# ChainSafe/lumenos

Measured on AMD Instinct MI355X. Metric: prove_eval_seconds_16384x4096, lower is better.
Workload: dtype u64; 1 GPU; Encode+Commit+InnerProduct(r,b)+QueryCols 16384x4096 LogN=14 L=12 K=2 rhoInv=2 queries=309; parallelism=1 GPU: the whole job resident in HBM

## Files before the change

### lumenos_amd/csrc/lm_common.h

```cpp
#pragma once
#include <hip/hip_runtime.h>

#include <algorithm>
#include <cstdarg>
#include <cstdint>
#include <cstdio>
#include <map>
#include <memory>
#include <mutex>
#include <set>
#include <string>
#include <utility>
#include <vector>

#include "../../include/lumenos_hip.h"
#include "lm_arith.h"
#include "lm_dev.h"

#define LM_MAX_LIMBS LUMEN_MAX_LIMBS

struct lm_modmap {
    uint32_t period;
    uint8_t idx[LM_MAX_LIMBS];
};

struct lm_mods {
    mod_t m[LM_MAX_LIMBS];
};

struct lm_prof_entry {
    double total_ms = 0;
    uint64_t launches = 0;
    uint64_t units = 0;
};

struct lm_galois_key {
    lm_dev<u64> d_key;
    lm_dev<uint32_t> d_index;
    lm_dev<uint32_t> d_inv_index;
};

struct lumen_set {
    uint32_t count = 0;
    uint32_t nl = 0;
    uint32_t logw = 0;
    u64 *d = nullptr;
    size_t words = 0;
    bool owner = true;
    lumen_ctx *home = nullptr;
};

struct lm_shared {
    std::recursive_mutex mu;
    lm_dev<tw_t> tw_fwd;
    lm_dev<tw_t> tw_inv;
    std::vector<uint64_t> roots;
    uint32_t fieldN = 0;
    lm_dev<tw_t> scal;
    std::map<uint64_t, lm_galois_key> gkeys;
    std::map<std::string, std::shared_ptr<void>> ext;
};

struct lm_tuning {
    uint32_t ks_batch = 64;
    uint32_t ks_lanes = 0;
    int32_t ks_fused_digits = -1;
    uint32_t ks_close_fused = 1;
    uint32_t ks_c0_fold = 1;
    uint32_t debug = 0;
    uint32_t modup_tgroup = 3, moddown_tgroup = 1;
    uint32_t ks_placement = 6;
    uint32_t batch_chunks = 0;
    uint32_t dot_pairs = 0;
    uint32_t dot_parts = 0;
    uint32_t rccl_shared_device = 0;
};

struct lumen_ctx {
    lm_tuning tune;
    std::recursive_mutex mu;
    std::shared_ptr<lm_shared> sh;
    int device = 0;
    hipStream_t stream = nullptr;
    hipStream_t stream2 = nullptr;
    hipEvent_t ev_fork = nullptr, ev_join = nullptr;
    hipStream_t stream_aux = nullptr;
    hipEvent_t ev_aux = nullptr;
    hipEvent_t ev_xdep = nullptr;
    uint32_t aux_digests = 0;
    const u64 *aux_lo = nullptr, *aux_hi = nullptr;
    uint8_t *aux_host = nullptr;
    size_t aux_host_cap = 0;
    void *stage_host = nullptr;
    size_t stage_cap = 0;
    hipEvent_t ev_stage = nullptr;
    void *io_host[2] = {nullptr, nullptr};
    hipEvent_t ev_io[2] = {nullptr, nullptr};
    uint32_t logN = 0, N = 0, L = 0, K = 0;
    uint64_t T = 0;
    uint64_t mod[LM_MAX_LIMBS] = {0};
    uint64_t psi[LM_MAX_LIMBS] = {0};
    lm_mods mods;
    tw_t ninv[LM_MAX_LIMBS];
    std::vector<uint64_t> &roots;
    uint32_t &fieldN;
    std::map<uint64_t, lm_galois_key> &gkeys;
    std::map<std::string, std::shared_ptr<void>> &ext;
    uint64_t mul_counter = 0;
    std::map<std::string, lm_dev<unsigned char>> scratch;
    struct pool_block {
        void *p;
        hipEvent_t ready;
    };
    std::multimap<size_t, pool_block> pool;
    size_t pool_bytes = 0;
    std::set<const void *> lds_attr_done;
    bool prof = false;
    std::map<std::string, lm_prof_entry> prof_tab;
    struct pending_ev {
        std::string name;
        hipEvent_t a, b;
        uint64_t units;
    };
    std::vector<pending_ev> prof_pending;
    std::vector<hipEvent_t> ev_pool;
    hipEvent_t tm0 = nullptr, tm1 = nullptr;
    std::string err;
    explicit lumen_ctx(std::shared_ptr<lm_shared> s)
        : sh(std::move(s)), roots(sh->roots), fieldN(sh->fieldN), gkeys(sh->gkeys), ext(sh->ext) {}
};

static inline size_t lm_ctw(const lumen_ctx *ctx, const lumen_set *s);
#define LM_FULL_WIDTH(ctx, set, what) \
    LM_CHECK(ctx, (set)->logw == 0, "%s: lane-sharded set (1/%u of every limb) where a full-width set is required", what, 1u << (set)->logw)

#define LM_ENTER(ctx)                                             \
    std::lock_guard<std::recursive_mutex> lm_lock_((ctx)->mu);    \
    (void)hipSetDevice((ctx)->device);                            \
    (void)hipGetLastError()
#define LM_SHARED_LOCK(ctx) std::lock_guard<std::recursive_mutex> lm_shlock_((ctx)->sh->mu)

template <class T>
static inline std::shared_ptr<T> lm_ext_get(lumen_ctx *ctx, const std::string &key) {
    LM_SHARED_LOCK(ctx);
    auto it = ctx->ext.find(key);
    return it == ctx->ext.end() ? std::shared_ptr<T>() : std::static_pointer_cast<T>(it->second);
}
static inline void lm_ext_put(lumen_ctx *ctx, const std::string &key, std::shared_ptr<void> v) {
    LM_SHARED_LOCK(ctx);
    ctx->ext[key] = std::move(v);
}

static inline size_t lm_ctw(const lumen_ctx *ctx, const lumen_set *s) { return (size_t)2 * s->nl * (ctx->N >> s->logw); }

void lm_sync_all(lumen_ctx *ctx);
void *lm_stage(lumen_ctx *ctx, size_t bytes);
int lm_h2d_staged(lumen_ctx *ctx, void *dev, const void *host, size_t bytes);
bool lm_host_is_pinned(const void *p);
int lm_h2d(lumen_ctx *ctx, void *dev, const void *host, size_t bytes);
int lm_d2h(lumen_ctx *ctx, void *host, const void *dev, size_t bytes, bool wait);
int lm_h2d_rows(lumen_ctx *ctx, void *dev, size_t dpitch, const void *host, size_t spitch, size_t width, size_t height);

int lm_fail(lumen_ctx *ctx, const char *fmt, ...);
extern thread_local std::string lm_global_err;

#define LM_HIP(ctx, call)                                                                  \
    do {                                                                                   \
        hipError_t e_ = (call);                                                            \
        if (e_ != hipSuccess)                                                              \
            return lm_fail(ctx, "%s failed: %s (%s:%d)", #call, hipGetErrorString(e_),     \
                           __FILE__, __LINE__);                                            \
    } while (0)

#define LM_CHECK(ctx, cond, ...)                    \
    do {                                            \
        if (!(cond)) return lm_fail(ctx, __VA_ARGS__); \
    } while (0)

template <class... P, class... A>
static inline int lm_launch_flat(lumen_ctx *ctx, void (*kernel)(P...), size_t threads, A &&...args) {
    hipLaunchKernelGGL(kernel, dim3((uint32_t)((threads + 255) / 256)), dim3(256), 0, ctx->stream, std::forward<A>(args)...);
    LM_HIP(ctx, hipGetLastError());
    return 0;
}

struct lm_set_guard {
    lumen_ctx *ctx;
    lumen_set *s;
    lm_set_guard(lumen_ctx *c, lumen_set *x) : ctx(c), s(x) {}
    ~lm_set_guard() {
        if (s) lumen_set_destroy(ctx, s);
    }
    lumen_set *release() {
        lumen_set *r = s;
        s = nullptr;
        return r;
    }
    lm_set_guard(lm_set_guard &&o) : ctx(o.ctx), s(o.release()) {}
    lm_set_guard &operator=(const lm_set_guard &) = delete;
};

void lm_set_release_async(lumen_ctx *ctx, lumen_set *set);

void *lm_scratch(lumen_ctx *ctx, const char *name, size_t bytes);
void lm_scratch_adopt(lumen_ctx *ctx, const char *name, void *p, size_t bytes);

struct lm_prof_scope {
    lumen_ctx *ctx;
    const char *name;
    uint64_t units;
    hipEvent_t a = nullptr;
    lm_prof_scope(lumen_ctx *c, const char *n, uint64_t u);
    ~lm_prof_scope();
};
void lm_prof_resolve(lumen_ctx *ctx);

static inline uint64_t h_mulmod(uint64_t a, uint64_t b, uint64_t q) {
    return (uint64_t)(((u128)a * b) % q);
}
static inline uint64_t h_powmod(uint64_t a, uint64_t e, uint64_t q) {
    uint64_t r = 1 % q;
    a %= q;
    while (e) {
        if (e & 1) r = h_mulmod(r, a, q);
        a = h_mulmod(a, a, q);
        e >>= 1;
    }
    return r;
}
static inline uint64_t h_invmod(uint64_t a, uint64_t q) { return h_powmod(a, q - 2, q); }
static inline tw_t h_tw(uint64_t w, uint64_t q) {
    tw_t t;
    t.w = w;
    t.wp = (u64)((((u128)w) << 64) / q);
    return t;
}
static inline uint64_t h_r64_mod(uint64_t q) { return (uint64_t)((((u128)1) << 64) % q); }
static inline uint64_t h_p_mod(const lumen_ctx *ctx, uint64_t q) {
    uint64_t P = 1 % q;
    for (uint32_t a = 0; a < ctx->K; a++) P = h_mulmod(P, ctx->mod[ctx->L + a] % q, q);
    return P;
}
static inline uint32_t h_bitrev(uint32_t x, int bits) {
    uint32_t r = 0;
    for (int i = 0; i < bits; i++) r = (r << 1) | ((x >> i) & 1);
    return r;
}

int lm_launch_ntt(lumen_ctx *ctx, u64 *d, uint32_t npoly, const lm_modmap &map, bool inverse);
struct lm_ninv_t;
int lm_launch_ntt_strided(lumen_ctx *ctx, const u64 *src, size_t src_poly_stride, u64 *dst,
                          size_t dst_poly_stride, uint32_t npoly, const lm_modmap &map, bool inverse,
                          const char *prof_name, const lm_ninv_t *inv_scale = nullptr);
int lm_launch_ntt_subring(lumen_ctx *ctx, uint32_t logn, const tw_t *tw, tw_t ninv_scale, const u64 *src,
                          size_t src_poly_stride, u64 *dst, size_t dst_poly_stride, uint32_t npoly,
                          uint32_t mod_idx, bool inverse, const mod_t *explicit_mod = nullptr);
mod_t lm_make_mod(uint64_t q);
void lm_build_tw(uint64_t q, uint64_t psi, uint32_t logN, std::vector<tw_t> &fwd, std::vector<tw_t> &inv);
int lm_rescale_polys(lumen_ctx *ctx, const u64 *src, uint32_t nl, u64 *dst, uint32_t target,
                     uint32_t npoly, u64 *work, u64 *tbuf);
int lm_rescale_coef_ready(lumen_ctx *ctx);
int lm_rescale_polys_from_coef(lumen_ctx *ctx, const u64 *coef, uint32_t nl, u64 *dst, uint32_t target, uint32_t npoly);
lm_modmap lm_map_q(uint32_t nl);
lm_modmap lm_map_p(const lumen_ctx *ctx);
int lm_encode_dev(lumen_ctx *ctx, const lumen_set *matrix, const u64 *dzero, uint32_t rho_inv, lumen_set **encoded);
int lm_poly_eval_check(lumen_ctx *ctx, const uint64_t *values, uint32_t rows, uint32_t count, uint64_t first_column,
                       uint32_t cols, const char *what);
int lm_poly_eval_enqueue(lumen_ctx *ctx, const uint64_t *values, uint32_t rows, uint32_t count, uint64_t first_column,
                         uint32_t cols, uint64_t z, const char *what);
int lm_poly_eval_finish(lumen_ctx *ctx, uint64_t *partial);
hipEvent_t lm_ev_get(lumen_ctx *ctx);
```

### lumenos_amd/csrc/lm_ctx.hip

```cpp
#include <cstring>
#include <thread>

#include "lm_ntt_plan.h"

thread_local std::string lm_global_err;

int lm_fail(lumen_ctx *ctx, const char *fmt, ...) {
    char buf[1024];
    va_list ap;
    va_start(ap, fmt);
    vsnprintf(buf, sizeof(buf), fmt, ap);
    va_end(ap);
    if (ctx) ctx->err = buf;
    lm_global_err = buf;
    fprintf(stderr, "[lumenos_hip] error: %s\n", buf);
    return 1;
}

void *lm_scratch(lumen_ctx *ctx, const char *name, size_t bytes) {
    auto &e = ctx->scratch[name];
    if (e && e.count() >= bytes) return e.get();
    if (e) lm_sync_all(ctx);
    return e.alloc(ctx, bytes, name) ? nullptr : e.get();
}

void lm_scratch_adopt(lumen_ctx *ctx, const char *name, void *p, size_t bytes) {
    auto &e = ctx->scratch[name];
    if (e.get() == p) (void)e.release();
    if (e) lm_sync_all(ctx);
    e = lm_dev<unsigned char>((unsigned char *)p, bytes);
}

void lm_sync_all(lumen_ctx *ctx) {
    if (ctx->stream) hipStreamSynchronize(ctx->stream);
    if (ctx->stream2) hipStreamSynchronize(ctx->stream2);
    if (ctx->stream_aux) hipStreamSynchronize(ctx->stream_aux);
}

void *lm_stage(lumen_ctx *ctx, size_t bytes) {
    if (ctx->ev_stage) hipEventSynchronize(ctx->ev_stage);
    if (ctx->stage_cap < bytes) {
        if (ctx->stage_host) hipHostFree(ctx->stage_host);
        ctx->stage_host = nullptr, ctx->stage_cap = 0;
        if (hipHostMalloc(&ctx->stage_host, bytes, hipHostMallocDefault) != hipSuccess) {
            lm_fail(ctx, "hipHostMalloc(%zu) for host staging failed", bytes);
            return nullptr;
        }
        ctx->stage_cap = bytes;
    }
    return ctx->stage_host;
}

int lm_h2d_staged(lumen_ctx *ctx, void *dev, const void *host, size_t bytes) {
    void *h = lm_stage(ctx, bytes);
    if (!h) return 1;
    memcpy(h, host, bytes);
    LM_HIP(ctx, hipMemcpyAsync(dev, h, bytes, hipMemcpyHostToDevice, ctx->stream));
    LM_HIP(ctx, hipEventRecord(ctx->ev_stage, ctx->stream));
    return 0;
}

hipEvent_t lm_ev_get(lumen_ctx *ctx) {
    if (!ctx->ev_pool.empty()) {
        hipEvent_t e = ctx->ev_pool.back();
        ctx->ev_pool.pop_back();
        return e;
    }
    hipEvent_t e = nullptr;
    hipEventCreate(&e);
    return e;
}

lm_prof_scope::lm_prof_scope(lumen_ctx *c, const char *n, uint64_t u) : ctx(c), name(n), units(u) {
    if (!ctx->prof) return;
    a = lm_ev_get(ctx);
    hipEventRecord(a, ctx->stream);
}
lm_prof_scope::~lm_prof_scope() {
    if (!ctx->prof || !a) return;
    hipEvent_t b = lm_ev_get(ctx);
    hipEventRecord(b, ctx->stream);
    ctx->prof_pending.push_back({name, a, b, units});
}

void lm_prof_resolve(lumen_ctx *ctx) {
    if (ctx->prof_pending.empty()) return;
    for (auto &p : ctx->prof_pending) {
        float ms = 0;
        if (hipEventSynchronize(p.b) == hipSuccess && hipEventElapsedTime(&ms, p.a, p.b) == hipSuccess) {
            auto &e = ctx->prof_tab[p.name];
            e.total_ms += ms;
            e.launches += 1;
            e.units += p.units;
        } else {
            (void)hipGetLastError();
        }
        ctx->ev_pool.push_back(p.a);
        ctx->ev_pool.push_back(p.b);
    }
    ctx->prof_pending.clear();
}

lm_modmap lm_map_q(uint32_t nl) {
    lm_modmap m;
    m.period = nl;
    for (uint32_t i = 0; i < LM_MAX_LIMBS; i++) m.idx[i] = (uint8_t)(i < nl ? i : 0);
    return m;
}

lm_modmap lm_map_p(const lumen_ctx *ctx) {
    lm_modmap m;
    m.period = ctx->K;
    for (uint32_t i = 0; i < LM_MAX_LIMBS; i++) m.idx[i] = (uint8_t)(ctx->L + (i < ctx->K ? i : 0));
    return m;
}

mod_t lm_make_mod(uint64_t q) {
    mod_t m;
    m.q = q;
    m.qinv64 = (u64)((((u128)1) << 64) / q);
    u64 inv = 1;
    for (int it = 0; it < 6; it++) inv *= 2 - (u64)q * inv;
    m.qneg = (u64)0 - inv;
    u64 r = h_r64_mod(q);
    m.r2 = h_mulmod(r, r, q);
    return m;
}

void lm_build_tw(uint64_t q, uint64_t psi, uint32_t logN, std::vector<tw_t> &fwd, std::vector<tw_t> &inv) {
    uint32_t N = 1u << logN;
    fwd.resize(N);
    inv.resize(N);
    uint64_t psi_inv = h_invmod(psi, q), cf = 1, cb = 1;
    for (uint32_t j = 0; j < N; j++) {
        uint32_t r = h_bitrev(j, (int)logN);
        fwd[r] = h_tw(cf, q);
        inv[r] = h_tw(cb, q);
        cf = h_mulmod(cf, psi, q);
        cb = h_mulmod(cb, psi_inv, q);
    }
}

static void pool_drain(lumen_ctx *ctx) {
    for (auto &kv : ctx->pool) {
        hipFree(kv.second.p);
        if (kv.second.ready) ctx->ev_pool.push_back(kv.second.ready);
    }
    ctx->pool.clear();
    ctx->pool_bytes = 0;
}

static int ctx_private_init(lumen_ctx *ctx) {
    LM_HIP(ctx, hipSetDevice(ctx->device));
    LM_HIP(ctx, hipStreamCreate(&ctx->stream));
    LM_HIP(ctx, hipStreamCreate(&ctx->stream2));
    LM_HIP(ctx, hipEventCreateWithFlags(&ctx->ev_fork, hipEventDisableTiming));
    LM_HIP(ctx, hipEventCreateWithFlags(&ctx->ev_join, hipEventDisableTiming));
    LM_HIP(ctx, hipStreamCreate(&ctx->stream_aux));
    LM_HIP(ctx, hipEventCreateWithFlags(&ctx->ev_aux, hipEventDisableTiming));
    LM_HIP(ctx, hipEventCreateWithFlags(&ctx->ev_stage, hipEventDisableTiming));
    LM_HIP(ctx, hipEventCreateWithFlags(&ctx->ev_xdep, hipEventDisableTiming));
    LM_HIP(ctx, hipEventCreate(&ctx->tm0));
    LM_HIP(ctx, hipEventCreate(&ctx->tm1));
    return 0;
}

static int tuning_set(lm_tuning &t, const char *name, long v) {
    const std::string n(name ? name : "");
    auto in = [&](long lo, long hi) { return v >= lo && v <= hi; };
    if (n == "LUMEN_KS_BATCH") {
        if (!in(1, 4096)) return 2;
        t.ks_batch = (uint32_t)v;
    } else if (n == "LUMEN_KS_LANES") {
        if (!in(0, 2)) return 2;
        t.ks_lanes = (uint32_t)v;
    } else if (n == "LUMEN_KS_FUSED_DIGITS") {
        if (v > LM_MAX_LIMBS) return 2;
        t.ks_fused_digits = v >= 0 ? (int32_t)v : -1;
    } else if (n == "LUMEN_KS_CLOSE_FUSED") {
        if (!in(0, 1)) return 2;
        t.ks_close_fused = (uint32_t)v;
    } else if (n == "LUMEN_KS_C0_FOLD") {
        if (!in(0, 1)) return 2;
        t.ks_c0_fold = (uint32_t)v;
    } else if (n == "LUMEN_DEBUG") {
        t.debug = v != 0;
    } else if (n == "LUMEN_MODUP_TGROUP") {
        if (!in(1, 31)) return 2;
        t.modup_tgroup = (uint32_t)v;
    } else if (n == "LUMEN_MODDOWN_TGROUP") {
        if (!in(1, 31)) return 2;
        t.moddown_tgroup = (uint32_t)v;
    } else if (n == "LUMEN_KS_PLACEMENT") {
        if (!in(0, 32)) return 2;
        t.ks_placement = (uint32_t)v;
    } else if (n == "LUMEN_BATCH_CHUNKS") {
        if (!in(0, 4096)) return 2;
        t.batch_chunks = (uint32_t)v;
    } else if (n == "LUMEN_DOT_PAIRS") {
        if (v != 0 && v != 256 && v != 512) return 2;
        t.dot_pairs = (uint32_t)v;
    } else if (n == "LUMEN_DOT_PARTS") {
        if (!in(0, 256)) return 2;
        t.dot_parts = (uint32_t)v;
    } else {
        return 1;
    }
    return 0;
}
static void tuning_from_env(lm_tuning &t) {
    for (const char *n : {"LUMEN_KS_BATCH", "LUMEN_KS_LANES", "LUMEN_KS_FUSED_DIGITS", "LUMEN_KS_CLOSE_FUSED", "LUMEN_KS_C0_FOLD", "LUMEN_DEBUG",
                          "LUMEN_MODUP_TGROUP", "LUMEN_MODDOWN_TGROUP", "LUMEN_KS_PLACEMENT", "LUMEN_BATCH_CHUNKS", "LUMEN_DOT_PAIRS", "LUMEN_DOT_PARTS"}) {
        const char *e = getenv(n);
        if (e && *e && tuning_set(t, n, atol(e)))
            fprintf(stderr, "[lumenos_hip] %s=%s is out of range: ignored\n", n, e);
    }
}

extern "C" int lumen_ctx_set_tuning(lumen_ctx *ctx, const char *name, long value) {
    LM_CHECK(nullptr, ctx && name, "lumen_ctx_set_tuning: NULL argument");
    LM_ENTER(ctx);
    const int rc = tuning_set(ctx->tune, name, value);
    LM_CHECK(ctx, rc != 1, "unknown tuning switch %s", name);
    LM_CHECK(ctx, rc == 0, "tuning switch %s: value %ld is out of range (nothing changed)", name, value);
    return 0;
}

extern "C" int lumen_test_allow_shared_device_rccl(lumen_ctx *ctx, int on) {
    LM_CHECK(nullptr, ctx, "lumen_test_allow_shared_device_rccl: NULL ctx");
    LM_ENTER(ctx);
    ctx->tune.rccl_shared_device = on != 0;
    return 0;
}

extern "C" int lumen_ctx_wait(lumen_ctx *ctx, lumen_ctx *other) {
    LM_CHECK(nullptr, ctx && other, "lumen_ctx_wait: NULL argument");
    if (ctx == other) return 0;
    hipEvent_t ev;
    {
        LM_ENTER(other);
        LM_HIP(other, hipEventRecord(other->ev_xdep, other->stream));
        ev = other->ev_xdep;
    }
    LM_ENTER(ctx);
    LM_CHECK(ctx, ctx->device == other->device, "lumen_ctx_wait: contexts on devices %d and %d", ctx->device, other->device);
    LM_HIP(ctx, hipStreamWaitEvent(ctx->stream, ev, 0));
    return 0;
}

extern "C" int lumen_ctx_create(const lumen_params_desc *desc, lumen_ctx **out) {
    if (!desc || !out) return lm_fail(nullptr, "lumen_ctx_create: NULL argument");
    *out = nullptr;
    LM_CHECK(nullptr, desc->abi_version == LUMEN_ABI_VERSION, "ABI version mismatch: got %u want %u",
             desc->abi_version, LUMEN_ABI_VERSION);
    LM_CHECK(nullptr, lm_logn_supported(desc->log_n) || lm_logn_split_supported(desc->log_n),
             "log_n %u unsupported: kernels are instantiated for N = 2^8 and 2^10..2^14, and the server's path and the key "
             "switch for N = 2^15",
             desc->log_n);
    LM_CHECK(nullptr, desc->num_q >= 1 && desc->num_q + desc->num_p <= LM_MAX_LIMBS,
             "bad limb counts L=%u K=%u", desc->num_q, desc->num_p);
    int ndev = 0;
    if (hipGetDeviceCount(&ndev) != hipSuccess || ndev == 0)
        return lm_fail(nullptr, "no HIP device visible: the lumenos HIP path has no CPU fallback");
    LM_CHECK(nullptr, desc->device >= 0 && desc->device < ndev, "device %d out of range (have %d)",
             desc->device, ndev);
    std::unique_ptr<lumen_ctx, void (*)(lumen_ctx *)> guard(new lumen_ctx(std::make_shared<lm_shared>()),
                                                            lumen_ctx_destroy);
    lumen_ctx *ctx = guard.get();
    tuning_from_env(ctx->tune);
    ctx->device = desc->device;
    ctx->logN = desc->log_n;
    ctx->N = 1u << desc->log_n;
    ctx->L = desc->num_q;
    ctx->K = desc->num_p;
    ctx->T = desc->plaintext_modulus;
    uint32_t LK = ctx->L + ctx->K, N = ctx->N;
    uint64_t two_n = 2ull * N;
    for (uint32_t i = 0; i < LK; i++) {
        uint64_t q = desc->moduli[i], psi = desc->psi[i];
        const uint64_t qmax = UINT64_MAX / lm_q_bound_factor(desc->log_n);
        if (q < (1ull << 20) || q > qmax || (q & (two_n - 1)) != 1)
            return lm_fail(nullptr, "modulus %u (%llu) must be == 1 mod 2N and below %llu", i,
                           (unsigned long long)q, (unsigned long long)qmax);
        if (h_powmod(psi, N, q) != q - 1)
            return lm_fail(nullptr, "psi[%u] is not a primitive 2N-th root of unity", i);
        ctx->mod[i] = q;
        ctx->psi[i] = psi;
        ctx->mods.m[i] = lm_make_mod(q);
        ctx->ninv[i] = h_tw(h_invmod(N % q, q), q);
    }
    for (uint32_t i = LK; i < LM_MAX_LIMBS; i++) ctx->mods.m[i] = ctx->mods.m[0];
    if (int rc = ctx_private_init(ctx)) return rc;
    std::vector<tw_t> f, b, fwd, inv;
    for (uint32_t i = 0; i < LK; i++) {
        lm_build_tw(ctx->mod[i], ctx->psi[i], ctx->logN, f, b);
        fwd.insert(fwd.end(), f.begin(), f.end());
        inv.insert(inv.end(), b.begin(), b.end());
    }
    lm_layout_tw(fwd, ctx->logN);
    lm_layout_tw(inv, ctx->logN);
    if (ctx->sh->tw_fwd.upload(ctx, fwd, "the forward twiddles") || ctx->sh->tw_inv.upload(ctx, inv, "the inverse twiddles")) return 1;
    *out = guard.release();
    return 0;
}

extern "C" int lumen_ctx_clone(lumen_ctx *src, lumen_ctx **out) {
    if (!src || !out) return lm_fail(nullptr, "lumen_ctx_clone: NULL argument");
    *out = nullptr;
    LM_ENTER(src);
    std::unique_ptr<lumen_ctx, void (*)(lumen_ctx *)> guard(new lumen_ctx(src->sh), lumen_ctx_destroy);
    lumen_ctx *ctx = guard.get();
    ctx->tune = src->tune;
    ctx->device = src->device;
    ctx->logN = src->logN, ctx->N = src->N, ctx->L = src->L, ctx->K = src->K, ctx->T = src->T;
    memcpy(ctx->mod, src->mod, sizeof(ctx->mod));
    memcpy(ctx->psi, src->psi, sizeof(ctx->psi));
    ctx->mods = src->mods;
    memcpy(ctx->ninv, src->ninv, sizeof(ctx->ninv));
    if (int rc = ctx_private_init(ctx)) {
        src->err = ctx->err;
        return rc;
    }
    *out = guard.release();
    return 0;
}

extern "C" void lumen_ctx_destroy(lumen_ctx *ctx) {
    if (!ctx) return;
    {
        LM_ENTER(ctx);
        lm_sync_all(ctx);
        ctx->scratch.clear();
        pool_drain(ctx);
        lm_prof_resolve(ctx);
        for (hipEvent_t e : ctx->ev_pool) hipEventDestroy(e);
        if (ctx->tm0) hipEventDestroy(ctx->tm0);
        if (ctx->tm1) hipEventDestroy(ctx->tm1);
        if (ctx->aux_host) hipHostFree(ctx->aux_host);
        if (ctx->stage_host) hipHostFree(ctx->stage_host);
        for (int i = 0; i < 2; i++) {
            if (ctx->io_host[i]) hipHostFree(ctx->io_host[i]);
            if (ctx->ev_io[i]) hipEventDestroy(ctx->ev_io[i]);
        }
        if (ctx->ev_stage) hipEventDestroy(ctx->ev_stage);
        if (ctx->ev_xdep) hipEventDestroy(ctx->ev_xdep);
        if (ctx->ev_aux) hipEventDestroy(ctx->ev_aux);
        if (ctx->stream_aux) hipStreamDestroy(ctx->stream_aux);
        if (ctx->ev_fork) hipEventDestroy(ctx->ev_fork);
        if (ctx->ev_join) hipEventDestroy(ctx->ev_join);
        if (ctx->stream2) hipStreamDestroy(ctx->stream2);
        if (ctx->stream) hipStreamDestroy(ctx->stream);
        ctx->sh.reset();
    }
    delete ctx;
}

extern "C" int lumen_ctx_trim(lumen_ctx *ctx) {
    LM_CHECK(nullptr, ctx, "lumen_ctx_trim: NULL ctx");
    LM_ENTER(ctx);
    LM_CHECK(ctx, !ctx->aux_digests, "lumen_ctx_trim: a lumen_leaf_digests_begin job is in flight");
    lm_sync_all(ctx);
    for (auto it = ctx->scratch.begin(); it != ctx->scratch.end();) {
        if (it->first == "digests_async" || it->first == "group_digests") {
            ++it;
            continue;
        }
        it = ctx->scratch.erase(it);
    }
    pool_drain(ctx);
    return 0;
}

extern "C" int lumen_ctx_scratch_info(lumen_ctx *ctx, const char *name, void **ptr, size_t *bytes) {
    LM_CHECK(nullptr, ctx && name && ptr, "lumen_ctx_scratch_info: NULL argument");
    LM_ENTER(ctx);
    auto it = ctx->scratch.find(name);
    *ptr = it == ctx->scratch.end() ? nullptr : it->second.get();
    if (bytes) *bytes = it == ctx->scratch.end() ? 0 : it->second.count();
    return 0;
}

extern "C" const char *lumen_last_error(const lumen_ctx *ctx) {
    return ctx ? ctx->err.c_str() : lm_global_err.c_str();
}

extern "C" int lumen_sync(lumen_ctx *ctx) {
    LM_CHECK(nullptr, ctx, "lumen_sync: NULL ctx");
    LM_ENTER(ctx);
    LM_HIP(ctx, hipStreamSynchronize(ctx->stream));
    return 0;
}

extern "C" uint64_t lumen_mul_counter(const lumen_ctx *ctx) { return ctx ? ctx->mul_counter : 0; }

extern "C" int lumen_set_create(lumen_ctx *ctx, uint32_t count, uint32_t num_limbs, lumen_set **out) {
    return lumen_set_create_lanes(ctx, count, num_limbs, 0, out);
}

extern "C" int lumen_set_create_lanes(lumen_ctx *ctx, uint32_t count, uint32_t num_limbs, uint32_t log_world,
                                      lumen_set **out) {
    LM_CHECK(nullptr, ctx && out, "lumen_set_create: NULL argument");
    LM_ENTER(ctx);
    LM_CHECK(ctx, num_limbs >= 1 && num_limbs <= ctx->L, "num_limbs %u out of range [1,%u]", num_limbs, ctx->L);
    LM_CHECK(ctx, log_world <= 6 && (ctx->N >> log_world) >= 64, "a lane shard of 1/%u of N = %u is narrower than 64 coefficients",
             1u << log_world, ctx->N);
    lumen_set *s = new lumen_set();
    s->count = count;
    s->nl = num_limbs;
    s->logw = log_world;
    s->words = (size_t)count * 2 * num_limbs * (ctx->N >> log_world);
    s->home = ctx;
    if (s->words) {
        const size_t bytes = s->words * sizeof(u64);
        auto it = ctx->pool.find(bytes);
        if (it != ctx->pool.end()) {
            s->d = (u64 *)it->second.p;
            if (hipEvent_t ready = it->second.ready) {
                (void)hipStreamWaitEvent(ctx->stream, ready, 0);
                (void)hipStreamWaitEvent(ctx->stream2, ready, 0);
                (void)hipStreamWaitEvent(ctx->stream_aux, ready, 0);
                ctx->ev_pool.push_back(ready);
            }
            ctx->pool.erase(it);
            ctx->pool_bytes -= bytes;
        } else {
            hipError_t e = hipMalloc((void **)&s->d, bytes);
            if (e != hipSuccess && !ctx->pool.empty()) {
                (void)hipGetLastError();
                lm_sync_all(ctx);
                pool_drain(ctx);
                e = hipMalloc((void **)&s->d, bytes);
            }
            if (e != hipSuccess) {
                (void)hipGetLastError();
                delete s;
                return lm_fail(ctx, "hipMalloc(%zu bytes) for a %u x %u-limb set failed: %s", bytes, count,
                               num_limbs, hipGetErrorString(e));
            }
        }
    }
    *out = s;
    return 0;
}

extern "C" void lumen_set_destroy(lumen_ctx *ctx, lumen_set *set) {
    if (!set) return;
    if (ctx) {
        LM_ENTER(ctx);
        hipStreamSynchronize(ctx->stream);
        hipStreamSynchronize(ctx->stream2);
        if (ctx->aux_digests && set->d && set->d < ctx->aux_hi && set->d + set->words > ctx->aux_lo)
            hipStreamSynchronize(ctx->stream_aux);
        if (set->owner && set->d) {
            const size_t bytes = set->words * sizeof(u64);
            if (ctx == set->home && ctx->pool_bytes + bytes <= ((size_t)96 << 30)) {
                ctx->pool.emplace(bytes, lumen_ctx::pool_block{set->d, nullptr});
                ctx->pool_bytes += bytes;
            } else {
                hipFree(set->d);
            }
        }
    } else if (set->owner && set->d) {
        hipFree(set->d);
    }
    delete set;
}

void lm_set_release_async(lumen_ctx *ctx, lumen_set *set) {
    if (!set) return;
    LM_ENTER(ctx);
    const size_t bytes = set->words * sizeof(u64);
    const bool hashing = ctx->aux_digests && set->d && set->d < ctx->aux_hi && set->d + set->words > ctx->aux_lo;
    if (!set->owner || !set->d || ctx != set->home || hashing || ctx->pool_bytes + bytes > ((size_t)96 << 30)) {
        lumen_set_destroy(ctx, set);
        return;
    }
    hipEvent_t ready = lm_ev_get(ctx);
    bool ok = ready && hipEventRecord(ctx->ev_join, ctx->stream2) == hipSuccess &&
              hipStreamWaitEvent(ctx->stream, ctx->ev_join, 0) == hipSuccess && hipEventRecord(ready, ctx->stream) == hipSuccess;
    if (!ok) {
        (void)hipGetLastError();
        if (ready) ctx->ev_pool.push_back(ready);
        lumen_set_destroy(ctx, set);
        return;
    }
    ctx->pool.emplace(bytes, lumen_ctx::pool_block{set->d, ready});
    ctx->pool_bytes += bytes;
    delete set;
}

extern "C" int lumen_set_slice(lumen_ctx *ctx, const lumen_set *set, uint32_t first, uint32_t n,
                               lumen_set **view) {
    LM_CHECK(nullptr, ctx && set && view, "lumen_set_slice: NULL argument");
    LM_ENTER(ctx);
    LM_CHECK(ctx, (uint64_t)first + n <= set->count, "slice [%u,%u) exceeds set of %u", first, first + n, set->count);
    lumen_set *v = new lumen_set();
    const size_t ctw = lm_ctw(ctx, set);
    v->count = n;
    v->nl = set->nl;
    v->logw = set->logw;
    v->d = set->d + (size_t)first * ctw;
    v->words = (size_t)n * ctw;
    v->owner = false;
    *view = v;
    return 0;
}

extern "C" uint32_t lumen_set_count(const lumen_set *set) { return set ? set->count : 0; }
extern "C" uint32_t lumen_set_limbs(const lumen_set *set) { return set ? set->nl : 0; }
extern "C" uint32_t lumen_set_log_world(const lumen_set *set) { return set ? set->logw : 0; }
extern "C" void *lumen_set_device_ptr(const lumen_set *set) { return set ? set->d : nullptr; }

extern "C" void *lumen_host_alloc(size_t bytes) {
    void *p = nullptr;
    if (hipHostMalloc(&p, bytes ? bytes : 1, hipHostMallocDefault) != hipSuccess) {
        (void)hipGetLastError();
        lm_fail(nullptr, "hipHostMalloc(%zu) failed", bytes);
        return nullptr;
    }
    return p;
}
extern "C" void lumen_host_free(void *p) {
    if (p) hipHostFree(p);
}

static int host_limbs_move(uint64_t *flat, uint64_t *const *limbs, size_t n, size_t words, uint32_t threads, bool gather) {
    if (!n || !words) return 0;
    const size_t bytes = words * sizeof(uint64_t);
    size_t nthr = threads ? threads : std::max(1u, std::min(16u, std::thread::hardware_concurrency()));
    nthr = std::min(nthr, n);
    auto work = [=](size_t lo, size_t hi) {
        for (size_t i = lo; i < hi; i++) {
            if (gather) memcpy(flat + i * words, limbs[i], bytes);
            else memcpy(limbs[i], flat + i * words, bytes);
        }
    };
    if (nthr == 1) {
        work(0, n);
        return 0;
    }
    std::vector<std::thread> th;
    for (size_t t = 0; t < nthr; t++) th.emplace_back(work, n * t / nthr, n * (t + 1) / nthr);
    for (auto &x : th) x.join();
    return 0;
}
extern "C" int lumen_host_gather(uint64_t *dst, const uint64_t *const *limbs, size_t n, size_t words, uint32_t threads) {
    LM_CHECK(nullptr, (dst && limbs) || !n, "lumen_host_gather: NULL argument");
    for (size_t i = 0; i < n; i++) LM_CHECK(nullptr, limbs[i], "lumen_host_gather: limb %zu is NULL", i);
    return host_limbs_move(dst, const_cast<uint64_t *const *>(limbs), n, words, threads, true);
}
extern "C" int lumen_host_scatter(const uint64_t *src, uint64_t *const *limbs, size_t n, size_t words, uint32_t threads) {
    LM_CHECK(nullptr, (src && limbs) || !n, "lumen_host_scatter: NULL argument");
    for (size_t i = 0; i < n; i++) LM_CHECK(nullptr, limbs[i], "lumen_host_scatter: limb %zu is NULL", i);
    return host_limbs_move(const_cast<uint64_t *>(src), limbs, n, words, threads, false);
}

bool lm_host_is_pinned(const void *p) {
    hipPointerAttribute_t a;
    if (hipPointerGetAttributes(&a, p) != hipSuccess) {
        (void)hipGetLastError();
        return false;
    }
    return a.type == hipMemoryTypeHost;
}

#define LM_IO_CHUNK ((size_t)64 << 20)
static void par_memcpy(void *dst, const void *src, size_t bytes) {
    const size_t nthr = bytes >= ((size_t)8 << 20) ? 4 : 1;
    if (nthr == 1) {
        memcpy(dst, src, bytes);
        return;
    }
    std::thread th[4];
    const size_t part = (bytes / nthr + 63) & ~(size_t)63;
    for (size_t t = 0; t < nthr; t++) {
        const size_t lo = std::min(bytes, t * part), hi = std::min(bytes, lo + part);
        th[t] = std::thread([=] { memcpy((char *)dst + lo, (const char *)src + lo, hi - lo); });
    }
    for (size_t t = 0; t < nthr; t++) th[t].join();
}

static int io_buffers(lumen_ctx *ctx) {
    for (int i = 0; i < 2; i++) {
        if (!ctx->io_host[i]) LM_HIP(ctx, hipHostMalloc(&ctx->io_host[i], LM_IO_CHUNK, hipHostMallocDefault));
        if (!ctx->ev_io[i]) LM_HIP(ctx, hipEventCreateWithFlags(&ctx->ev_io[i], hipEventDisableTiming));
    }
    return 0;
}

int lm_h2d(lumen_ctx *ctx, void *dev, const void *host, size_t bytes) {
    char *dst = (char *)dev;
    if (bytes <= ((size_t)1 << 20) || lm_host_is_pinned(host)) {
        LM_HIP(ctx, hipMemcpyAsync(dst, host, bytes, hipMemcpyHostToDevice, ctx->stream));
    } else {
        if (int rc = io_buffers(ctx)) return rc;
        int i = 0;
        for (size_t off = 0; off < bytes; off += LM_IO_CHUNK, i ^= 1) {
            const size_t len = std::min(LM_IO_CHUNK, bytes - off);
            LM_HIP(ctx, hipEventSynchronize(ctx->ev_io[i]));
            par_memcpy(ctx->io_host[i], (const char *)host + off, len);
            LM_HIP(ctx, hipMemcpyAsync(dst + off, ctx->io_host[i], len, hipMemcpyHostToDevice, ctx->stream));
            LM_HIP(ctx, hipEventRecord(ctx->ev_io[i], ctx->stream));
        }
    }
    LM_HIP(ctx, hipStreamSynchronize(ctx->stream));
    return 0;
}

int lm_h2d_rows(lumen_ctx *ctx, void *dev, size_t dpitch, const void *host, size_t spitch, size_t width, size_t height) {
    char *dst = (char *)dev;
    const char *src = (const char *)host;
    if (!width || !height) return 0;
    if (width * height <= ((size_t)1 << 20) || lm_host_is_pinned(host)) {
        LM_HIP(ctx, hipMemcpy2DAsync(dst, dpitch, src, spitch, width, height, hipMemcpyHostToDevice, ctx->stream));
    } else {
        LM_CHECK(ctx, width <= LM_IO_CHUNK, "lm_h2d_rows: a row of %zu bytes exceeds the bounce buffer", width);
        if (int rc = io_buffers(ctx)) return rc;
        const size_t per = LM_IO_CHUNK / width;
        int i = 0;
        for (size_t r = 0; r < height; r += per, i ^= 1) {
            const size_t nr = std::min(per, height - r);
            LM_HIP(ctx, hipEventSynchronize(ctx->ev_io[i]));
            if (spitch == width)
                par_memcpy(ctx->io_host[i], src + r * spitch, nr * width);
            else
                for (size_t k = 0; k < nr; k++) memcpy((char *)ctx->io_host[i] + k * width, src + (r + k) * spitch, width);
            LM_HIP(ctx, hipMemcpy2DAsync(dst + r * dpitch, dpitch, ctx->io_host[i], width, width, nr, hipMemcpyHostToDevice,
                                         ctx->stream));
            LM_HIP(ctx, hipEventRecord(ctx->ev_io[i], ctx->stream));
        }
    }
    LM_HIP(ctx, hipStreamSynchronize(ctx->stream));
    return 0;
}

extern "C" int lumen_set_upload(lumen_ctx *ctx, lumen_set *set, uint32_t first, uint32_t n,
                                const uint64_t *host) {
    LM_CHECK(nullptr, ctx && set && host, "lumen_set_upload: NULL argument");
    LM_ENTER(ctx);
    LM_CHECK(ctx, (uint64_t)first + n <= set->count, "upload range [%u,%u) exceeds set of %u", first, first + n, set->count);
    const size_t ctw = lm_ctw(ctx, set), bytes = (size_t)n * ctw * sizeof(u64);
    return lm_h2d(ctx, set->d + (size_t)first * ctw, host, bytes);
}

int lm_d2h(lumen_ctx *ctx, void *host, const void *dev, size_t bytes, bool wait) {
    const char *src = (const char *)dev;
    if (bytes <= ((size_t)1 << 20) || lm_host_is_pinned(host)) {
        LM_HIP(ctx, hipMemcpyAsync(host, src, bytes, hipMemcpyDeviceToHost, ctx->stream));
        if (wait || !lm_host_is_pinned(host)) LM_HIP(ctx, hipStreamSynchronize(ctx->stream));
        return 0;
    }
    if (int rc = io_buffers(ctx)) return rc;
    const size_t nchunks = (bytes + LM_IO_CHUNK - 1) / LM_IO_CHUNK;
    auto issue = [&](size_t k) -> int {
        const size_t off = k * LM_IO_CHUNK, len = std::min(LM_IO_CHUNK, bytes - off);
        LM_HIP(ctx, hipMemcpyAsync(ctx->io_host[k & 1], src + off, len, hipMemcpyDeviceToHost, ctx->stream));
        LM_HIP(ctx, hipEventRecord(ctx->ev_io[k & 1], ctx->stream));
        return 0;
    };
    if (nchunks)
        if (int rc = issue(0)) return rc;
    for (size_t k = 0; k < nchunks; k++) {
        if (k + 1 < nchunks)
            if (int rc = issue(k + 1)) return rc;
        const size_t off = k * LM_IO_CHUNK, len = std::min(LM_IO_CHUNK, bytes - off);
        LM_HIP(ctx, hipEventSynchronize(ctx->ev_io[k & 1]));
        par_memcpy((char *)host + off, ctx->io_host[k & 1], len);
    }
    return 0;
}

extern "C" int lumen_set_download(lumen_ctx *ctx, const lumen_set *set, uint32_t first, uint32_t n,
                                  uint64_t *host) {
    LM_CHECK(nullptr, ctx && set && host, "lumen_set_download: NULL argument");
    LM_ENTER(ctx);
    LM_CHECK(ctx, (uint64_t)first + n <= set->count, "download range [%u,%u) exceeds set of %u", first, first + n, set->count);
    const size_t ctw = lm_ctw(ctx, set), bytes = (size_t)n * ctw * sizeof(u64);
    return lm_d2h(ctx, host, set->d + (size_t)first * ctw, bytes, true);
}

__global__ void k_fill_random(u64 *d, size_t words, uint32_t N, uint32_t nl, lm_mods mods, u64 seed) {
    size_t i = (size_t)blockIdx.x * blockDim.x + threadIdx.x;
    size_t stride = (size_t)gridDim.x * blockDim.x;
    for (; i < words; i += stride) {
        uint32_t limb = (uint32_t)((i / N) % nl);
        u64 z = seed + 0x9e3779b97f4a7c15ull * (u64)(i + 1);
        z = (z ^ (z >> 30)) * 0xbf58476d1ce4e5b9ull;
        z = (z ^ (z >> 27)) * 0x94d049bb133111ebull;
        z ^= z >> 31;
        d[i] = lm_reduce(z, mods.m[limb].q, mods.m[limb].qinv64);
    }
}

extern "C" int lumen_set_fill_random(lumen_ctx *ctx, lumen_set *set, uint64_t seed) {
    LM_CHECK(nullptr, ctx && set, "lumen_set_fill_random: NULL argument");
    LM_ENTER(ctx);
    if (!set->words) return 0;
    hipLaunchKernelGGL(k_fill_random, dim3(2048), dim3(256), 0, ctx->stream, set->d, set->words,
                       ctx->N >> set->logw, set->nl, ctx->mods, (u64)seed);
    LM_HIP(ctx, hipGetLastError());
    return 0;
}

extern "C" int lumen_timer_start(lumen_ctx *ctx) {
    LM_CHECK(nullptr, ctx, "NULL ctx");
    LM_ENTER(ctx);
    LM_HIP(ctx, hipEventRecord(ctx->tm0, ctx->stream));
    return 0;
}

extern "C" int lumen_timer_stop(lumen_ctx *ctx, float *elapsed_ms) {
    LM_CHECK(nullptr, ctx && elapsed_ms, "NULL argument");
    LM_ENTER(ctx);
    LM_HIP(ctx, hipEventRecord(ctx->tm1, ctx->stream));
    LM_HIP(ctx, hipEventSynchronize(ctx->tm1));
    LM_HIP(ctx, hipEventElapsedTime(elapsed_ms, ctx->tm0, ctx->tm1));
    return 0;
}

extern "C" int lumen_prof_enable(lumen_ctx *ctx, int on) {
    LM_CHECK(nullptr, ctx, "NULL ctx");
    LM_ENTER(ctx);
    if (!on) lm_prof_resolve(ctx);
    ctx->prof = on != 0;
    return 0;
}

extern "C" int lumen_prof_reset(lumen_ctx *ctx) {
    LM_CHECK(nullptr, ctx, "NULL ctx");
    LM_ENTER(ctx);
    lm_prof_resolve(ctx);
    ctx->prof_tab.clear();
    return 0;
}

extern "C" size_t lumen_prof_names(lumen_ctx *ctx, char *buf, size_t cap) {
    if (!ctx) return 0;
    LM_ENTER(ctx);
    lm_prof_resolve(ctx);
    std::string all;
    for (auto &kv : ctx->prof_tab) {
        if (!all.empty()) all += ",";
        all += kv.first;
    }
    if (buf && cap) {
        size_t n = std::min(cap - 1, all.size());
        memcpy(buf, all.data(), n);
        buf[n] = 0;
    }
    return all.size();
}

extern "C" int lumen_prof_read(lumen_ctx *ctx, const char *kernel, double *total_ms,
                               uint64_t *launches, uint64_t *units) {
    LM_CHECK(nullptr, ctx && kernel, "NULL argument");
    LM_ENTER(ctx);
    lm_prof_resolve(ctx);
    auto it = ctx->prof_tab.find(kernel);
    lm_prof_entry e;
    if (it != ctx->prof_tab.end()) e = it->second;
    if (total_ms) *total_ms = e.total_ms;
    if (launches) *launches = e.launches;
    if (units) *units = e.units;
    return 0;
}
```

### lumenos_amd/csrc/lm_innersum.hip

```cpp
#include <algorithm>

#include "lm_ks_host.h"

__global__ __launch_bounds__(256) void k_acc_canon(u64 *__restrict__ acc, size_t pairs, uint32_t logN, uint32_t L, lm_mods mods) {
    const size_t stride = (size_t)gridDim.x * blockDim.x;
    for (size_t g = (size_t)blockIdx.x * blockDim.x + threadIdx.x; g < pairs; g += stride) {
        const u64 q = mods.m[(uint32_t)((g >> (logN - 1)) % L)].q;
        ulonglong2 v = *reinterpret_cast<ulonglong2 *>(acc + 2 * g);
        v.x = lm_csub(v.x, q), v.y = lm_csub(v.y, q);
        *reinterpret_cast<ulonglong2 *>(acc + 2 * g) = v;
    }
}

__global__ __launch_bounds__(256) void k_lazy_gather(const u64 *__restrict__ u, const u64 *__restrict__ cur, u64 *__restrict__ lazy,
                                                     const uint32_t *__restrict__ index, uint32_t B, uint32_t L, uint32_t K,
                                                     uint32_t pshift, uint32_t logN, uint32_t first, lm_mods mods) {
    const uint32_t N = 1u << logN, nq = L * 2 * B;
    const size_t total = (size_t)2 * B * (L + K) * (N / 2), stride = (size_t)gridDim.x * blockDim.x;
    for (size_t g = (size_t)blockIdx.x * blockDim.x + threadIdx.x; g < total; g += stride) {
        const uint32_t j = (uint32_t)(g & (N / 2 - 1)) * 2, limb = (uint32_t)(g >> (logN - 1));
        const uint32_t t = limb < nq ? limb / (2 * B) : L + (limb - nq) % K;
        const uint32_t pw = limb < nq ? limb % (2 * B) : (limb - nq) / K;
        const bool with_c = t < L && (pw & 1) == (u ? 0u : 1u);
        if (!u && !with_c) continue;
        const u64 q = mods.m[ks_mod_at(t, L, pshift)].q;
        const size_t o = ((size_t)limb << logN) + j;
        uint2 p;
        p.x = j, p.y = j + 1;
        if (index) p = *reinterpret_cast<const uint2 *>(index + j);
        ulonglong2 v;
        v.x = v.y = 0;
        if (!first) v = *reinterpret_cast<const ulonglong2 *>(lazy + o);
        if (u) v.x += u[((size_t)limb << logN) + p.x], v.y += u[((size_t)limb << logN) + p.y];
        if (with_c) {
            const u64 *c = cur + (((size_t)pw * L + t) << logN);
            v.x += c[p.x], v.y += c[p.y];
        }
        v.x = lm_csub(lm_csub(v.x, 2 * q), q), v.y = lm_csub(lm_csub(v.y, 2 * q), q);
        *reinterpret_cast<ulonglong2 *>(lazy + o) = v;
    }
}

namespace {

int acc_canon(lumen_ctx *ctx, u64 *acc, size_t words, uint32_t L) {
    if (!words) return 0;
    hipLaunchKernelGGL(k_acc_canon, dim3(2048), dim3(256), 0, ctx->stream, acc, words / 2, ctx->logN, L, ctx->mods);
    LM_HIP(ctx, hipGetLastError());
    return 0;
}


bool is_plain(const lumen_ctx *ctx, uint32_t batch, uint32_t n) { return batch == 1 && n && !(n & (n - 1)) && n <= ctx->N; }

template <class Fn>
int sum_walk(const lumen_ctx *ctx, uint32_t batch, uint32_t n, Fn &&fn) {
    if (is_plain(ctx, batch, n)) {
        uint64_t gal[64];
        const uint32_t cnt = lumen_inner_sum_galois_elements(ctx, n, gal);
        for (uint32_t r = 0; r < cnt; r++)
            if (int rc = fn((uint64_t)0, gal[r])) return rc;
        return 0;
    }
    for (uint32_t i = 0, j = n; j > 1; i++, j >>= 1) {
        const uint64_t term = (j & 1) ? lumen_galois_element(ctx, (int64_t)((uint64_t)(n - (n & ((2u << i) - 1))) * batch)) : 0;
        if (int rc = fn(term, lumen_galois_element(ctx, (int64_t)((uint64_t)batch << i)))) return rc;
    }
    return 0;
}

struct SumPlan {
    struct Step {
        const lm_galois_key *dbl = nullptr, *term = nullptr;
        uint64_t dbl_el = 0;
    } it[32];
    uint32_t cnt = 0;
    uint64_t last_el = 0;
    bool lazy = false;
};

int sum_plan(lumen_ctx *ctx, uint32_t batch, uint32_t n, SumPlan *p) {
    return sum_walk(ctx, batch, n, [&](uint64_t term, uint64_t dbl) {
        SumPlan::Step &st = p->it[p->cnt++];
        if (term) {
            if (int rc = ks_find_key(ctx, term, &st.term)) return rc;
            p->lazy = true;
        }
        p->last_el = st.dbl_el = dbl;
        return ks_find_key(ctx, dbl, &st.dbl);
    });
}

int general_check(lumen_ctx *ctx, uint32_t batch, uint32_t n, const char *what) {
    LM_CHECK(ctx, batch >= 1 && n >= 1, "%s: batch size %u and length %u must both be at least 1", what, batch, n);
    LM_CHECK(ctx, ctx->K >= 1, "parameters have no special primes: key switching unavailable");
    LM_CHECK(ctx, ctx->K <= 2, "key switching supports 1 or 2 special primes (have %u)", ctx->K);
    if (is_plain(ctx, batch, n)) return 0;
    LM_CHECK(ctx, (uint64_t)batch * n <= ctx->N / 2, "%s: batch size %u x length %u spans beyond the slot row of %u slots", what, batch, n,
             ctx->N / 2);
    return 0;
}

}


int lazy_blocks(lumen_ctx *ctx, const KsRun &run, u64 **lazy) {
    const size_t bytes = (size_t)run.Bmax * 2 * (ctx->L + ctx->K) * ctx->N * 8;
    lazy[0] = (u64 *)lm_scratch(ctx, "ks_lazy", bytes);
    lazy[1] = run.lanes > 1 ? (u64 *)lm_scratch(ctx, "ks_lazy_b", bytes) : lazy[0];
    return lazy[0] && lazy[1] ? 0 : 1;
}

static int lazy_gather(lumen_ctx *ctx, const u64 *u, const u64 *cur, u64 *lazy, const uint32_t *index, bool first, uint32_t B, KsTables *tb) {
    lm_prof_scope ps(ctx, "ks_lazy_gather", (uint64_t)B);
    hipLaunchKernelGGL(k_lazy_gather, dim3(2048), dim3(256), 0, ctx->stream, u, cur, lazy, index, B, tb->nl, ctx->K, ctx->L - tb->nl,
                       ctx->logN, first ? 1u : 0u, ctx->mods);
    LM_HIP(ctx, hipGetLastError());
    return 0;
}

int identity_tables(lumen_ctx *ctx, std::shared_ptr<lm_galois_key> *out) {
    static const char *const NAME = "ks_identity";
    LM_SHARED_LOCK(ctx);
    auto gk = lm_ext_get<lm_galois_key>(ctx, NAME);
    if (!gk) {
        gk = std::make_shared<lm_galois_key>();
        std::vector<uint32_t> index(ctx->N);
        for (uint32_t i = 0; i < ctx->N; i++) index[i] = i;
        if (gk->d_index.upload(ctx, index, "the identity's index table") || gk->d_inv_index.upload(ctx, index, "the identity's index table"))
            return 1;
        lm_ext_put(ctx, NAME, gk);
    }
    *out = std::move(gk);
    return 0;
}

int lazy_close(lumen_ctx *ctx, const u64 *cur, u64 *out, u64 *lazy, uint32_t B, KsTables *tb, const KsScratch &s) {
    std::shared_ptr<lm_galois_key> id;
    if (int rc = identity_tables(ctx, &id)) return rc;
    if (int rc = lazy_gather(ctx, nullptr, cur, lazy, nullptr, false, B, tb)) return rc;
    if (int rc = rotate_p_to_coef(ctx, lazy, B, tb)) return rc;
    KsScratch sl = s;
    sl.u = lazy;
    return rotate_store(ctx, cur, out, B, *id, tb, sl);
}

namespace {

int inner_sum_batch(lumen_ctx *ctx, u64 *acc, uint32_t B, const SumPlan &plan, KsTables *tb, const KsScratch &s, u64 *lazy,
                    u64 *close_out, u64 *fold_s = nullptr) {
    LM_CHECK(ctx, !close_out || (plan.cnt && !plan.lazy), "InnerSum has no rotation to close");
    LM_CHECK(ctx, !fold_s || (close_out && ks_fold_serves(ctx, tb, plan.cnt)),
             "the c0 fold cannot hold the lifts of %u rotations of %u bits in 192", plan.cnt, tb->lift_bits);
    u64 *cur = acc, *other = s.acc2;
    bool first = true;
    for (uint32_t r = 0; r < plan.cnt; r++) {
        const SumPlan::Step &st = plan.it[r];
        if (int rc = rotate_decompose(ctx, cur, B, tb, s)) return rc;
        if (fold_s) {
            const u64 *s_in = r ? fold_s + ((r - 1) & 1) * ks_fold_words(ctx, B) : nullptr;
            u64 *s_out = fold_s + (r & 1) * ks_fold_words(ctx, B);
            if (r + 1 == plan.cnt) return rotate_close_fold(ctx, cur, close_out, B, *st.dbl, st.dbl_el, tb, s, s_in, s_out);
            if (int rc = rotate_add_fold(ctx, cur, other, B, *st.dbl, st.dbl_el, tb, s, s_in, s_out)) return rc;
            std::swap(cur, other);
            continue;
        }
        if (st.term) {
            if (int rc = rotate_mac(ctx, cur, B, *st.term, tb, s)) return rc;
            if (int rc = lazy_gather(ctx, s.u, cur, lazy, st.term->d_index.get(), first, B, tb)) return rc;
            first = false;
        }
        if (close_out && r + 1 == plan.cnt)
            return rotate_close(ctx, cur, close_out, B, *st.dbl, plan.last_el, tb, s);
        if (int rc = rotate_add(ctx, cur, other, B, *st.dbl, tb, s)) return rc;
        std::swap(cur, other);
    }
    if (plan.lazy) {
        if (int rc = lazy_close(ctx, cur, other, lazy, B, tb, s)) return rc;
        std::swap(cur, other);
    }
    if (cur != acc)
        LM_HIP(ctx, hipMemcpyAsync(acc, cur, (size_t)B * 2 * tb->nl * ctx->N * 8, hipMemcpyDeviceToDevice, ctx->stream));
    return 0;
}

int check_inner_sum_level(lumen_ctx *ctx, const lumen_set *in, const char *what) {
    LM_FULL_WIDTH(ctx, in, what);
    LM_CHECK(ctx, in->nl == ctx->L, "%s is implemented at the top level only (set has %u of %u limbs)", what,
             in->nl, ctx->L);
    return 0;
}

int inner_sum_run(lumen_ctx *ctx, const lumen_set *in, uint32_t batch, uint32_t n, const char *general, lumen_set **out) {
    if (general) {
        if (int rc = general_check(ctx, batch, n, general)) return rc;
    } else {
        LM_CHECK(ctx, is_plain(ctx, batch, n), "InnerSum length %u is not a power of two <= N", n);
    }
    KsRun run;
    if (int rc = ks_run_open(ctx, in->count, in->nl, is_plain(ctx, batch, n) ? 1 : 2, false, &run)) return rc;
    SumPlan plan;
    if (in->count)
        if (int rc = sum_plan(ctx, batch, n, &plan)) return rc;
    lumen_set *o = nullptr;
    if (int rc = lumen_set_create(ctx, in->count, in->nl, &o)) return rc;
    lm_set_guard og(ctx, o);
    if (in->words)
        LM_HIP(ctx, hipMemcpyAsync(o->d, in->d, in->words * 8, hipMemcpyDeviceToDevice, ctx->stream));
    if (int rc = ks_run_scratch(ctx, &run)) return rc;
    u64 *lazy[2] = {nullptr, nullptr};
    if (plan.lazy)
        if (int rc = lazy_blocks(ctx, run, lazy)) return rc;
    const size_t ctw = (size_t)2 * in->nl * ctx->N;
    auto batch_fn = [&](uint32_t, uint32_t first, uint32_t B, const KsScratch &s, u64 *) {
        return inner_sum_batch(ctx, o->d + (size_t)first * ctw, B, plan, run.tb, s, lazy[&s == &run.s[1]], nullptr);
    };
    if (int rc = ks_run(ctx, run, in->count, ctw, batch_fn)) return rc;
    if (!plan.lazy)
        if (int rc = acc_canon(ctx, o->d, o->words, in->nl)) return rc;
    *out = og.release();
    return 0;
}

int matrix_inner_sum_run(lumen_ctx *ctx, const lumen_set *matrix, const uint64_t *pt, uint32_t rows, const char *general,
                         lumen_set **out) {
    if (general) {
        if (int rc = general_check(ctx, 1, rows, general)) return rc;
    } else {
        LM_CHECK(ctx, is_plain(ctx, 1, rows), "rows=%u is not a power of two <= N", rows);
    }
    KsRun run;
    if (int rc = ks_run_open(ctx, matrix->count, matrix->nl, 2, true, &run)) return rc;
    SumPlan plan;
    if (matrix->count)
        if (int rc = sum_plan(ctx, 1, rows, &plan)) return rc;
    u64 *ptT = nullptr;
    if (int rc = upload_ptT(ctx, pt, matrix->nl, &ptT)) return rc;
    const uint32_t N = ctx->N, L = matrix->nl, target = std::min<uint32_t>(2, L);
    lumen_set *o = nullptr;
    if (int rc = lumen_set_create(ctx, matrix->count, target, &o)) return rc;
    lm_set_guard og(ctx, o);
    const size_t ctw = (size_t)2 * L * N, octw = (size_t)2 * target * N;
    if (int rc = ks_run_scratch(ctx, &run)) return rc;
    u64 *lazy[2] = {nullptr, nullptr};
    if (plan.lazy)
        if (int rc = lazy_blocks(ctx, run, lazy)) return rc;
    u64 *work = (u64 *)lm_scratch(ctx, "rescale_work", run.group_bytes);
    u64 *tbuf = (u64 *)lm_scratch(ctx, "rescale_t", (size_t)run.group * 2 * N * 8);
    if (!work || !tbuf) return 1;
    bool close = false;
    if (L > target && rows > 1 && ctx->tune.ks_close_fused && !plan.lazy && !lm_is_split(ctx->logN)) {
        const int rc = lm_rescale_coef_ready(ctx);
        if (rc && rc != 2) return rc;
        close = rc == 0;
    }
    u64 *fold_s[2] = {nullptr, nullptr};
    if (close && ctx->tune.ks_c0_fold && ks_fold_serves(ctx, run.tb, plan.cnt)) {
        const size_t bytes = 2 * ks_fold_words(ctx, run.Bmax) * 8;
        fold_s[0] = (u64 *)lm_scratch(ctx, "ks_fold_s", bytes);
        fold_s[1] = run.lanes > 1 ? (u64 *)lm_scratch(ctx, "ks_fold_s_b", bytes) : fold_s[0];
        if (!fold_s[0] || !fold_s[1]) return 1;
    }
    auto batch_fn = [&](uint32_t g0, uint32_t first, uint32_t B, const KsScratch &s, u64 *a) {
        if (int rc = launch_mul_plain(ctx, matrix->d + (size_t)(g0 + first) * ctw, a, ptT, (size_t)B * ctw, L, B))
            return rc;
        const int lane = &s == &run.s[1];
        return inner_sum_batch(ctx, a, B, plan, run.tb, s, lazy[lane], close ? work + (size_t)first * ctw : nullptr, fold_s[lane]);
    };
    auto end_of_group = [&](uint32_t g0, uint32_t gn) {
        if (close)
            return lm_rescale_polys_from_coef(ctx, work, L, o->d + (size_t)g0 * octw, target, gn * 2);
        if (L > target) return lm_rescale_polys(ctx, run.acc, L, o->d + (size_t)g0 * octw, target, gn * 2, work, tbuf);
        if (!plan.lazy)
            if (int rc = acc_canon(ctx, run.acc, (size_t)gn * ctw, L)) return rc;
        LM_HIP(ctx, hipMemcpyAsync(o->d + (size_t)g0 * octw, run.acc, (size_t)gn * ctw * 8, hipMemcpyDeviceToDevice, ctx->stream));
        return 0;
    };
    if (int rc = ks_run(ctx, run, matrix->count, ctw, batch_fn, end_of_group)) return rc;
    *out = og.release();
    return 0;
}

}

extern "C" int lumen_inner_sum_general(lumen_ctx *ctx, const lumen_set *in, uint32_t batch_size, uint32_t n, lumen_set **out) {
    LM_CHECK(nullptr, ctx && in && out, "lumen_inner_sum_general: NULL argument");
    LM_ENTER(ctx);
    if (int rc = check_level_of_chain(ctx, in, "InnerSum")) return rc;
    return inner_sum_run(ctx, in, batch_size, n, "lumen_inner_sum_general", out);
}

extern "C" int lumen_matrix_inner_sum_general(lumen_ctx *ctx, const lumen_set *matrix, const uint64_t *pt, uint32_t rows,
                                              lumen_set **out) {
    LM_CHECK(nullptr, ctx && matrix && pt && out, "lumen_matrix_inner_sum_general: NULL argument");
    LM_ENTER(ctx);
    if (int rc = check_level_of_chain(ctx, matrix, "matrixInnerSumEval")) return rc;
    return matrix_inner_sum_run(ctx, matrix, pt, rows, "lumen_matrix_inner_sum_general", out);
}

extern "C" uint32_t lumen_inner_sum_general_elements(const lumen_ctx *ctx, uint32_t batch_size, uint32_t n, uint64_t *gal_els) {
    if (!ctx || !gal_els) return 0;
    if (!is_plain(ctx, batch_size, n) && (!batch_size || !n || (uint64_t)batch_size * n > ctx->N / 2)) return 0;
    uint32_t cnt = 0;
    sum_walk(ctx, batch_size, n, [&](uint64_t term, uint64_t dbl) {
        for (uint64_t g : {term, dbl})
            if (g > 1 && std::find(gal_els, gal_els + cnt, g) == gal_els + cnt) gal_els[cnt++] = g;
        return 0;
    });
    return cnt;
}

extern "C" int lumen_inner_sum(lumen_ctx *ctx, const lumen_set *in, uint32_t n, lumen_set **out) {
    LM_CHECK(nullptr, ctx && in && out, "lumen_inner_sum: NULL argument");
    LM_ENTER(ctx);
    if (int rc = check_inner_sum_level(ctx, in, "InnerSum")) return rc;
    return inner_sum_run(ctx, in, 1, n, nullptr, out);
}

extern "C" int lumen_inner_sum_at_level(lumen_ctx *ctx, const lumen_set *in, uint32_t n, lumen_set **out) {
    LM_CHECK(nullptr, ctx && in && out, "lumen_inner_sum_at_level: NULL argument");
    LM_ENTER(ctx);
    if (int rc = check_level_of_chain(ctx, in, "InnerSum")) return rc;
    return inner_sum_run(ctx, in, 1, n, nullptr, out);
}

extern "C" int lumen_matrix_inner_sum(lumen_ctx *ctx, const lumen_set *matrix, const uint64_t *pt,
                                      uint32_t rows, lumen_set **out) {
    LM_CHECK(nullptr, ctx && matrix && pt && out, "lumen_matrix_inner_sum: NULL argument");
    LM_ENTER(ctx);
    if (int rc = check_inner_sum_level(ctx, matrix, "matrixInnerSumEval")) return rc;
    return matrix_inner_sum_run(ctx, matrix, pt, rows, nullptr, out);
}

extern "C" int lumen_matrix_inner_sum_at_level(lumen_ctx *ctx, const lumen_set *matrix, const uint64_t *pt,
                                               uint32_t rows, lumen_set **out) {
    LM_CHECK(nullptr, ctx && matrix && pt && out, "lumen_matrix_inner_sum_at_level: NULL argument");
    LM_ENTER(ctx);
    if (int rc = check_level_of_chain(ctx, matrix, "matrixInnerSumEval")) return rc;
    return matrix_inner_sum_run(ctx, matrix, pt, rows, nullptr, out);
}
```

### lumenos_amd/csrc/lm_keyswitch.hip

```cpp
#include <cstdlib>
#include <cstring>

#include "lm_ks_host.h"

__device__ __forceinline__ u32 bx_v(u128 A, u128 M, u64 y0, u64 y1, u64 m0, u64 m1) {
    const u128 D1 = A >= M ? A - M : M - A, D2 = 2 * M - A;
    if ((u64)(D1 >> 64) >= 8 && (u64)(D2 >> 64) >= 8) return A >= M ? 1u : 0u;
    double vf = 0.0;
    vf += (double)y0 / (double)m0;
    vf += (double)y1 / (double)m1;
    return (u32)(u64)vf;
}

__device__ __forceinline__ void pack_pair(u64 a, u64 b, u64 m0, u64 m1, u128 M, u64 &hi, u64 &lo) {
    u64 l1, h1, l2, h2;
    mul128(a, m1, l1, h1);
    mul128(b, m0, l2, h2);
    const u128 A = (((u128)h1 << 64) | l1) + (((u128)h2 << 64) | l2);
    const u32 v = bx_v(A, M, a, b, m0, m1);
    const u128 W = A + (v == 0 ? 2 * M : (v == 1 ? M : (u128)0));
    hi = (u64)(W >> LM_W_SPLIT), lo = (u64)W & ((1ull << LM_W_SPLIT) - 1);
}

__global__ __launch_bounds__(256) void k_pack_v(u64 *__restrict__ y, size_t poly_stride, uint32_t npoly,
                                                uint32_t ngroups, uint32_t group_limbs, uint32_t first_mod,
                                                uint32_t nlimbs_total, uint32_t logN, lm_mods mods) {
    const uint32_t N = 1u << logN;
    const size_t total = (size_t)npoly * ngroups * (N / 2), stride = (size_t)gridDim.x * blockDim.x;
    for (size_t g = (size_t)blockIdx.x * blockDim.x + threadIdx.x; g < total; g += stride) {
        const uint32_t i = (uint32_t)(g & (N / 2 - 1)) * 2;
        const uint32_t grp = (uint32_t)((g >> (logN - 1)) % ngroups), p = (uint32_t)((g >> (logN - 1)) / ngroups);
        const uint32_t l0 = grp * group_limbs;
        if (l0 + 1 >= nlimbs_total) continue;
        u64 *y0 = y + (size_t)p * poly_stride + (size_t)l0 * N + i;
        const ulonglong2 av = *reinterpret_cast<const ulonglong2 *>(y0);
        const ulonglong2 bv = *reinterpret_cast<const ulonglong2 *>(y0 + N);
        const u64 m0 = mods.m[first_mod + l0].q, m1 = mods.m[first_mod + l0 + 1].q;
        u64 Ml, Mh;
        mul128(m0, m1, Ml, Mh);
        const u128 M = ((u128)Mh << 64) | Ml;
        ulonglong2 hv, lv;
#pragma unroll
        for (int e = 0; e < 2; e++) {
            const u64 a = e ? av.y : av.x, b = e ? bv.y : bv.x;
            u64 hi, lo;
            pack_pair(a, b, m0, m1, M, hi, lo);
            if (e) hv.y = hi, lv.y = lo;
            else hv.x = hi, lv.x = lo;
        }
        *reinterpret_cast<ulonglong2 *>(y0) = hv;
        *reinterpret_cast<ulonglong2 *>(y0 + N) = lv;
    }
}

template <int LOGN>
__global__ LM_GEOM_BOUNDS(lm_geom_lds(LOGN)) void k_intt_pack(const u64 *__restrict__ acc, u64 *coef, uint32_t B,
                                                                  uint32_t L, uint32_t nf, lm_mods mods,
                                                                  lm_ninv_t yscale, const tw_t *__restrict__ tw_all) {
    extern __shared__ __attribute__((aligned(16))) u64 sm[];
    constexpr uint32_t N = 1u << LOGN;
    const uint32_t tid = threadIdx.x;
    if (blockIdx.x >= B * nf) {
        const uint32_t k = blockIdx.x - B * nf, l = 2 * nf + k / B, b = k % B;
        const u64 *p = acc + (((size_t)b * 2 + 1) * L + l) * N;
        u64 *o = coef + ((size_t)b * L + l) * N;
        const lm_qc q = lm_make_qc(mods.m[l]);
        const tw_t sc = yscale.t[l];
        auto ld = [&](uint32_t i0, u64 *v, int count) { lm_load_run(p, i0, v, count); };
        auto st = [&](uint32_t i, u64 v) { o[i] = lm_shoup_cs(v, sc, q.q, q.nq); };
        lm_ntt_inverse<LOGN>(sm, tw_all + (size_t)l * N, q, tid, ld, st);
        return;
    }
    const uint32_t d = blockIdx.x / B, b = blockIdx.x % B;
    const uint32_t l0 = 2 * d, l1 = l0 + 1;
    const u64 *c1 = acc + ((size_t)b * 2 + 1) * L * N;
    u64 *o0 = coef + ((size_t)b * L + l0) * N;
    const lm_qc q0 = lm_make_qc(mods.m[l0]);
    const tw_t s0 = yscale.t[l0];
    {
        const u64 *p = c1 + (size_t)l0 * N;
        auto ld = [&](uint32_t i0, u64 *v, int count) { lm_load_run(p, i0, v, count); };
        auto st = [&](uint32_t i, u64 v) { o0[i] = lm_shoup_cs(v, s0, q0.q, q0.nq); };
        lm_ntt_inverse<LOGN>(sm, tw_all + (size_t)l0 * N, q0, tid, ld, st);
    }
    __syncthreads();
    {
        const lm_qc q1 = lm_make_qc(mods.m[l1]);
        const tw_t s1 = yscale.t[l1];
        const u64 *p = c1 + (size_t)l1 * N;
        u64 Ml, Mh;
        mul128(q0.q, q1.q, Ml, Mh);
        auto uni = [](u64 x) {
            return (u64)(uint32_t)__builtin_amdgcn_readfirstlane((int)(uint32_t)x) |
                   (u64)(uint32_t)__builtin_amdgcn_readfirstlane((int)(uint32_t)(x >> 32)) << 32;
        };
        const u128 M = ((u128)uni(Mh) << 64) | uni(Ml);
        auto ld = [&](uint32_t i0, u64 *v, int count) { lm_load_run(p, i0, v, count); };
        constexpr int R_LAST = lm_pass_r(LOGN, 0), LOG_T0 = LOGN - R_LAST;
        constexpr int PF = (1 << R_LAST) * 5 / 8;
        struct pack_t {
            u64 *o0;
            const lm_qc &q0, &q1;
            tw_t s1;
            u128 M;
            u64 y0[PF];
            __device__ __forceinline__ void pre(uint32_t w) {
#pragma unroll
                for (int k = 0; k < PF; k++) y0[k] = o0[w + ((uint32_t)k << LOG_T0)];
            }
            __device__ __forceinline__ void operator()(uint32_t i, u64 v, int k) {
                const u64 y1 = lm_shoup_cs(v, s1, q1.q, q1.nq);
                uint32_t j = i;
                asm volatile("" : "+v"(j));
                const u64 a = k < PF ? y0[k < PF ? k : 0] : o0[j];
                u64 hi, lo;
                pack_pair(a, y1, q0.q, q1.q, M, hi, lo);
                o0[j] = hi, o0[j + N] = lo;
                if (k >= PF && (k & 1)) asm volatile("" ::: "memory");
            }
        } st{o0, q0, q1, s1, M, {}};
        uint32_t tid1 = tid;
        asm volatile("" : "+v"(tid1));
        lm_ntt_inverse<LOGN>(sm, tw_all + (size_t)l1 * N, q1, tid1, ld, st);
    }
}

template <int LOGN>
__global__ LM_GEOM_BOUNDS(lm_geom_fwd(LOGN)) void k_modup_ntt(const u64 *__restrict__ coef, const u64 *__restrict__ acc,
                                                    u64 *__restrict__ ext, const bx_t *__restrict__ bx,
                                                    uint32_t B, uint32_t L, uint32_t K, uint32_t beta, uint32_t pshift,
                                                    const uint32_t *__restrict__ work, lm_mods mods,
                                                    const tw_t *__restrict__ tw_all) {
    extern __shared__ __attribute__((aligned(16))) u64 sm[];
    constexpr uint32_t N = 1u << LOGN;
    const uint32_t tid = threadIdx.x, LK = L + K;
    const lm_half<LOGN> hf = lm_half_of_block<LOGN>();
    const uint32_t wk = work[hf.block];
    const uint32_t b = wk & 0xFFFF, d = (wk >> 16) & 0xFF, t = wk >> 24;
    const uint32_t mt = ks_mod_at(t, L, pshift);
    const bx_t c = bx[d * LK + t];
    u64 *o = ext + ks_ext_at(b, d, t, B, beta) * N + hf.off;
    const lm_qc qc = lm_make_qc(mods.m[mt]);
    const u64 *s0 = coef + ((size_t)b * L + d * K) * N;
    const u64 *s1 = c.ns == 2 ? s0 + N : s0;
    auto ld = [&](uint32_t i) { return bx_apply(c, s0[i], s1[i], qc); };
    auto out = [&](uint32_t j, u64 v0, u64 v1) {
        ulonglong2 y;
        y.x = v0, y.y = v1;
        *reinterpret_cast<ulonglong2 *>(o + j) = y;
    };
    if constexpr (LOGN == 14) {
        lm_w14_runs st{sm};
        auto after = [&](uint32_t i0, uint32_t) { lm_w14_linear_out(sm, tid, i0, out); };
        lm_ntt_forward_w14(sm, tw_all + (size_t)mt * N, qc, tid, ld, st, after);
    } else {
        lm_lds_runs st{sm};
        auto after = [&](uint32_t, uint32_t) { lm_linear_out<lm_tlog(LOGN)>(sm, tid, out); };
        lm_ntt_forward_half<LOGN>(sm, tw_all + (size_t)mt * N, qc, tid, hf, ld, st, after);
    }
}

#ifndef LM_MAC_COLS
#define LM_MAC_COLS 4
#endif
#ifndef LM_MAC_VEC
#define LM_MAC_VEC 1
#endif
#ifndef LM_MAC_PREFETCH
#define LM_MAC_PREFETCH 1
#endif
template <int VEC>
struct mac_vec;
template <>
struct mac_vec<1> {
    u64 v[1];
    static __device__ __forceinline__ mac_vec load(const u64 *p) { return mac_vec{{*p}}; }
    static __device__ __forceinline__ mac_vec load_once(const u64 *p) { return mac_vec{{__builtin_nontemporal_load(p)}}; }
    __device__ __forceinline__ void store(u64 *p) const { *p = v[0]; }
};
template <>
struct mac_vec<2> {
    u64 v[2];
    static __device__ __forceinline__ mac_vec load(const u64 *p) {
        const ulonglong2 a = *reinterpret_cast<const ulonglong2 *>(p);
        return mac_vec{{a.x, a.y}};
    }
    static __device__ __forceinline__ mac_vec load_once(const u64 *p) {
        return mac_vec{{__builtin_nontemporal_load(p), __builtin_nontemporal_load(p + 1)}};
    }
    __device__ __forceinline__ void store(u64 *p) const {
        ulonglong2 a;
        a.x = v[0], a.y = v[1];
        *reinterpret_cast<ulonglong2 *>(p) = a;
    }
};
struct mac_acc {
    u64 a0, a1, a3;
    u32 c0, c1;
    __device__ __forceinline__ void clear() { a0 = a1 = a3 = 0, c0 = c1 = 0; }
    __device__ __forceinline__ void value(u64 &lo, u64 &hi) const {
        lo = a0 + (a1 << 32);
        hi = a3 + c0 + (a1 >> 32) + ((u64)c1 << 32) + (lo < a0 ? 1 : 0);
    }
};
__device__ __forceinline__ void mac2(mac_acc &p, mac_acc &q, u64 x, u64 k0, u64 k1) {
    const u32 x0 = (u32)x, x1 = (u32)(x >> 32);
#if LM_ASM_SHOUP
    asm("v_mad_u64_u32 %[pa0], s[98:99], %[x0], %[k00], %[pa0]\n\t"
        "v_mad_u64_u32 %[qa0], s[90:91], %[x0], %[k10], %[qa0]\n\t"
        "v_mad_u64_u32 %[pa1], s[94:95], %[x0], %[k01], %[pa1]\n\t"
        "v_addc_co_u32_e64 %[pc0], s[96:97], %[pc0], 0, s[98:99]\n\t"
        "v_mad_u64_u32 %[qa1], s[92:93], %[x0], %[k11], %[qa1]\n\t"
        "v_addc_co_u32_e64 %[qc0], s[96:97], %[qc0], 0, s[90:91]\n\t"
        "v_mad_u64_u32 %[pa3], s[96:97], %[x1], %[k01], %[pa3]\n\t"
        "v_addc_co_u32_e64 %[pc1], s[96:97], %[pc1], 0, s[94:95]\n\t"
        "v_mad_u64_u32 %[pa1], s[98:99], %[x1], %[k00], %[pa1]\n\t"
        "v_addc_co_u32_e64 %[qc1], s[96:97], %[qc1], 0, s[92:93]\n\t"
        "v_mad_u64_u32 %[qa1], s[90:91], %[x1], %[k10], %[qa1]\n\t"
        "v_mad_u64_u32 %[qa3], s[96:97], %[x1], %[k11], %[qa3]\n\t"
        "v_addc_co_u32_e64 %[pc1], s[96:97], %[pc1], 0, s[98:99]\n\t"
        "v_addc_co_u32_e64 %[qc1], s[96:97], %[qc1], 0, s[90:91]"
        : [pa0] "+v"(p.a0), [pa1] "+v"(p.a1), [pa3] "+v"(p.a3), [pc0] "+v"(p.c0), [pc1] "+v"(p.c1),
          [qa0] "+v"(q.a0), [qa1] "+v"(q.a1), [qa3] "+v"(q.a3), [qc0] "+v"(q.c0), [qc1] "+v"(q.c1)
        : [x0] "v"(x0), [x1] "v"(x1), [k00] "v"((u32)k0), [k01] "v"((u32)(k0 >> 32)), [k10] "v"((u32)k1),
          [k11] "v"((u32)(k1 >> 32))
        : "s92", "s93", "s94", "s95", "s96", "s97", "s98", "s99", "s90", "s91");
#else
    auto one = [&](mac_acc &r, u64 k) {
        const u32 k0w = (u32)k, k1w = (u32)(k >> 32);
        u64 t = r.a0 + (u64)x0 * k0w;
        r.c0 += t < r.a0, r.a0 = t;
        t = r.a1 + (u64)x0 * k1w;
        r.c1 += t < r.a1, r.a1 = t;
        t = r.a1 + (u64)x1 * k0w;
        r.c1 += t < r.a1, r.a1 = t;
        r.a3 += (u64)x1 * k1w;
    };
    one(p, k0);
    one(q, k1);
#endif
}

#define LM_KS_MAC_FOLD 0
#include "lm_ks_mac_kernel.h"
#undef LM_KS_MAC_FOLD
#define LM_KS_MAC_FOLD 1
#include "lm_ks_mac_kernel.h"
#undef LM_KS_MAC_FOLD

template <int LOGN, bool ACCUMULATE>
__device__ __forceinline__ void moddown_body(const u64 *__restrict__ u, const u64 *__restrict__ acc_in,
                                             u64 *__restrict__ acc_out, const bx_t *__restrict__ bxp,
                                             const tw_t *__restrict__ pinv,
                                             const uint32_t *__restrict__ index,
                                             const uint32_t *__restrict__ inv_index,
                                             const uint32_t *__restrict__ work, uint32_t B,
                                             uint32_t L, uint32_t K, const lm_mods &mods,
                                             const tw_t *__restrict__ tw_all) {
    extern __shared__ __attribute__((aligned(16))) u64 sm[];
    constexpr uint32_t N = 1u << LOGN;
    const uint32_t tid = threadIdx.x;
    const lm_half<LOGN> hf = lm_half_of_block<LOGN>();
    const uint32_t wk = work[hf.block];
    const uint32_t pw = wk & 0xFFFF;
    const uint32_t t = wk >> 16;
    const uint32_t w = pw & 1;
    const bx_t c = bxp[t];
    const lm_qc qc = lm_make_qc(mods.m[t]);
    const u64 *up0 = u + ks_u_at(pw, L, B, L, K) * N;
    const u64 *up1 = c.ns == 2 ? up0 + N : up0;
    const u64 *uq = u + ks_u_at(pw, t, B, L, K) * N;
    const u64 *ain = acc_in + ((size_t)pw * L + t) * N;
    u64 *aout = acc_out + ((size_t)pw * L + t) * N;
    tw_t pi = pinv[t];
    pi.w = qc.q - pi.w, pi.wp = ~pi.wp;
    auto ld = [&](uint32_t i) { return bx_apply(c, up0[i], up1[i], qc); };
    if constexpr (LOGN == 14) {
        const uint32_t wave = tid >> 6, lane = tid & 63;
        const uint32_t jb0 = (uint32_t)__builtin_amdgcn_readfirstlane((int)(inv_index[(2 * wave) << 10] >> 10));
        const uint32_t jb1 = (uint32_t)__builtin_amdgcn_readfirstlane((int)(inv_index[(2 * wave + 1) << 10] >> 10));
        lm_w14_runs st{sm};
        auto after = [&](uint32_t i0h, uint32_t) {
            const uint32_t pb = LM_PAD((wave << 10) | (2 * lane));
            constexpr uint32_t CH = 4;
            const uint32_t i = (wave << 11) | i0h | (2 * lane);
            const uint32_t jb = i0h ? jb1 : jb0, sbase = wave << 10;
#pragma unroll
            for (uint32_t k0 = 0; k0 < 8; k0 += CH) {
                ulonglong2 uv[CH], cv[CH];
#pragma unroll
                for (uint32_t k = 0; k < CH; k++) {
                    uv[k] = *reinterpret_cast<const ulonglong2 *>(uq + i + 128 * (k0 + k));
                    if (w == 0) cv[k] = *reinterpret_cast<const ulonglong2 *>(ain + i + 128 * (k0 + k));
                }
#pragma unroll
                for (uint32_t k = 0; k < CH; k++) {
                    const uint32_t p = lm_w14_at(pb, 128 * (k0 + k));
                    const u64 a0 = w == 0 ? uv[k].x + cv[k].x : uv[k].x, a1 = w == 0 ? uv[k].y + cv[k].y : uv[k].y;
                    sm[p] = lm_shoup3<true>(sm[p], pi.w, pi.wp, qc.nq, a0);
                    sm[p + 1] = lm_shoup3<true>(sm[p + 1], pi.w, pi.wp, qc.nq, a1);
                }
                LM_W14_FENCE();
            }
            lm_wave_sync();
            uint2 p[8];
            ulonglong2 x[8];
#pragma unroll
            for (uint32_t k = 0; k < 8; k++) {
                const uint32_t j = (jb << 10) + 2 * lane + k * 128;
                p[k] = *reinterpret_cast<const uint2 *>(index + j);
                if constexpr (ACCUMULATE) x[k] = *reinterpret_cast<const ulonglong2 *>(ain + j);
            }
#pragma unroll
            for (uint32_t k = 0; k < 8; k++) {
                const uint32_t j = (jb << 10) + 2 * lane + k * 128;
                ulonglong2 y;
                if constexpr (ACCUMULATE) {
                    y.x = lm_csub(lm_csub(x[k].x + sm[LM_PAD(sbase | (p[k].x & 1023u))], 4 * qc.q), 2 * qc.q);
                    y.y = lm_csub(lm_csub(x[k].y + sm[LM_PAD(sbase | (p[k].y & 1023u))], 4 * qc.q), 2 * qc.q);
                } else {
                    y.x = lm_csub(lm_csub(lm_csub(sm[LM_PAD(sbase | (p[k].x & 1023u))], 4 * qc.q), 2 * qc.q), qc.q);
                    y.y = lm_csub(lm_csub(lm_csub(sm[LM_PAD(sbase | (p[k].y & 1023u))], 4 * qc.q), 2 * qc.q), qc.q);
                }
                *reinterpret_cast<ulonglong2 *>(aout + j) = y;
            }
        };
        lm_ntt_forward_w14(sm, tw_all + (size_t)t * N, qc, tid, ld, st, after);
    } else {
        constexpr int TLOG = lm_tlog(LOGN);
        constexpr int RUN = lm_fwd_run<TLOG>();
        static_assert(RUN <= 8, "lm_load_run moves at most 8 coefficients");
        struct storer_t {
            const u64 *uq, *ain;
            u64 *sm;
            const lm_qc &qc;
            tw_t pi;
            uint32_t w;
            u64 uv[RUN], cv[RUN];
            __device__ __forceinline__ void pre(uint32_t i0) {
                lm_load_run(uq, i0, uv, RUN);
                if (w == 0) lm_load_run(ain, i0, cv, RUN);
            }
            __device__ __forceinline__ void operator()(uint32_t i0, const u64 *v, int count) {
#pragma unroll
                for (int k = 0; k < RUN; k++)
                    if (k < count) {
                        const u64 add = w == 0 ? uv[k] + cv[k] : uv[k];
                        sm[LM_PAD(i0 + k)] = lm_shoup3<true>(v[k], pi.w, pi.wp, qc.nq, add);
                    }
            }
        } st{uq + hf.off, ain + hf.off, sm, qc, pi, w, {}, {}};
        constexpr uint32_t NW = lm_nthreads(TLOG) / 64, BLK = (1u << TLOG) / NW, IT = BLK / 128;
        const uint32_t wave = tid >> 6, lane = tid & 63;
        const uint32_t jb = NW > 1 ? (uint32_t)__builtin_amdgcn_readfirstlane((int)(inv_index[hf.off + wave * BLK] / BLK)) : 0u;
        auto after = [&](uint32_t, uint32_t) {
            uint2 p[IT];
            ulonglong2 x[IT];
#pragma unroll
            for (uint32_t k = 0; k < IT; k++) {
                const uint32_t j = jb * BLK + 2 * lane + k * 128;
                p[k] = *reinterpret_cast<const uint2 *>(index + j);
                if constexpr (ACCUMULATE) x[k] = *reinterpret_cast<const ulonglong2 *>(ain + j);
            }
            lm_wave_sync();
#pragma unroll
            for (uint32_t k = 0; k < IT; k++) {
                const uint32_t j = jb * BLK + 2 * lane + k * 128;
                ulonglong2 y;
                if constexpr (ACCUMULATE) {
                    y.x = lm_csub(lm_csub(x[k].x + sm[LM_PAD(lm_half_local<LOGN>(p[k].x))], 4 * qc.q), 2 * qc.q);
                    y.y = lm_csub(lm_csub(x[k].y + sm[LM_PAD(lm_half_local<LOGN>(p[k].y))], 4 * qc.q), 2 * qc.q);
                } else {
                    y.x = lm_csub(lm_csub(lm_csub(sm[LM_PAD(lm_half_local<LOGN>(p[k].x))], 4 * qc.q), 2 * qc.q), qc.q);
                    y.y = lm_csub(lm_csub(lm_csub(sm[LM_PAD(lm_half_local<LOGN>(p[k].y))], 4 * qc.q), 2 * qc.q), qc.q);
                }
                *reinterpret_cast<ulonglong2 *>(aout + j) = y;
            }
        };
        lm_ntt_forward_half<LOGN>(sm, tw_all + (size_t)t * N, qc, tid, hf, ld, st, after);
    }
}

#define LM_MODDOWN_PARAMS                                                                                                      \
    const u64 *__restrict__ u, const u64 *__restrict__ acc_in, u64 *__restrict__ acc_out, const bx_t *__restrict__ bxp,        \
        const tw_t *__restrict__ pinv, const uint32_t *__restrict__ index, const uint32_t *__restrict__ inv_index,             \
        const uint32_t *__restrict__ work, uint32_t B, uint32_t L, uint32_t K, lm_mods mods, const tw_t *__restrict__ tw_all
template <int LOGN>
__global__ LM_GEOM_BOUNDS(lm_geom_fwd(LOGN)) void k_moddown_ntt(LM_MODDOWN_PARAMS) {
    moddown_body<LOGN, true>(u, acc_in, acc_out, bxp, pinv, index, inv_index, work, B, L, K, mods, tw_all);
}
template <int LOGN>
__global__ LM_GEOM_BOUNDS(lm_geom_fwd(LOGN)) void k_rotdown_ntt(LM_MODDOWN_PARAMS) {
    moddown_body<LOGN, false>(u, acc_in, acc_out, bxp, pinv, index, inv_index, work, B, L, K, mods, tw_all);
}

namespace {

bx_t make_bx(const uint64_t *src, uint32_t ns, uint64_t t) {
    bx_t c;
    memset(&c, 0, sizeof(c));
    c.ns = ns;
    uint64_t m_mod_t = 1;
    for (uint32_t a = 0; a < ns; a++) m_mod_t = h_mulmod(m_mod_t, src[a] % t, t);
    c.b57 = h_tw((1ull << LM_W_SPLIT) % t, t);
    c.c_t = (t - h_mulmod(2 % t, m_mod_t, t)) % t;
    return c;
}

uint64_t hat_inv(const uint64_t *src, uint32_t ns, uint32_t a) {
    uint64_t h = 1;
    for (uint32_t b = 0; b < ns; b++)
        if (b != a) h = h_mulmod(h, src[b] % src[a], src[a]);
    return h_invmod(h, src[a]);
}

}

int get_tables(lumen_ctx *ctx, KsTables **out) { return get_tables_at(ctx, ctx->L, out); }

int get_tables_at(lumen_ctx *ctx, uint32_t nl, KsTables **out) {
    LM_SHARED_LOCK(ctx);
    LM_CHECK(ctx, nl >= 1 && nl <= ctx->L, "key switch at %u limbs: the chain has %u", nl, ctx->L);
    const std::string name = nl == ctx->L ? std::string("ks_tables") : "ks_tables:" + std::to_string(nl);
    auto it = ctx->ext.find(name);
    if (it != ctx->ext.end()) {
        *out = static_cast<KsTables *>(it->second.get());
        return 0;
    }
    const uint32_t L = nl, K = ctx->K, LK = L + K, pshift = ctx->L - nl, ctxLK = ctx->L + K;
    LM_CHECK(ctx, K >= 1 && K <= 2, "key switching supports 1 or 2 special primes (have %u)", K);
    auto sp = std::make_shared<KsTables>();
    KsTables &tb = *sp;
    tb.nl = L;
    tb.beta = (L + K - 1) / K;
    std::vector<bx_t> bx((size_t)tb.beta * LK);
    for (uint32_t d = 0; d < tb.beta; d++) {
        const uint32_t lo = d * K, hi = std::min(lo + K, L), ns = hi - lo;
        for (uint32_t t = 0; t < LK; t++) {
            bx_t c = make_bx(ctx->mod + lo, ns, ctx->mod[ks_mod_at(t, L, pshift)]);
            c.own = (t >= lo && t < hi) ? 1 : 0;
            bx[(size_t)d * LK + t] = c;
        }
    }
    for (uint32_t i = 0; i < LM_MAX_LIMBS; i++) tb.yscale.t[i] = ctx->ninv[i < ctxLK ? i : 0];
    for (uint32_t d = 0; d < tb.beta; d++) {
        const uint32_t lo = d * K, hi = std::min(lo + K, L), ns = hi - lo;
        for (uint32_t a = 0; a < ns; a++) {
            const uint64_t m = ctx->mod[lo + a];
            tb.yscale.t[lo + a] = h_tw(h_mulmod(ctx->ninv[lo + a].w, hat_inv(ctx->mod + lo, ns, a), m), m);
        }
    }
    for (uint32_t a = 0; a < K; a++) {
        const uint64_t m = ctx->mod[ctx->L + a];
        tb.yscale.t[ctx->L + a] = h_tw(h_mulmod(ctx->ninv[ctx->L + a].w, hat_inv(ctx->mod + ctx->L, K, a), m), m);
    }
    std::vector<bx_t> bxp(L);
    std::vector<tw_t> pinv(L);
    for (uint32_t t = 0; t < L; t++) {
        bxp[t] = make_bx(ctx->mod + ctx->L, K, ctx->mod[t]);
        const uint64_t q = ctx->mod[t];
        pinv[t] = h_tw(h_invmod(h_p_mod(ctx, q), q), q);
    }
    {
        unsigned __int128 M = 1;
        for (uint32_t a = 0; a < K; a++) M *= ctx->mod[ctx->L + a];
        const unsigned __int128 bound = K == 2 ? 2 * M : M;
        tb.m2_lo = K == 2 ? (u64)(2 * M) : 0, tb.m2_hi = K == 2 ? (u64)((2 * M) >> 64) : 0;
        for (tb.lift_bits = 0; tb.lift_bits < 128 && (bound >> tb.lift_bits); tb.lift_bits++) {}
    }
    std::vector<sfold_t> sfold(L);
    for (uint32_t t = 0; t < L; t++) {
        const uint64_t q = ctx->mod[t];
        const uint64_t r63 = (1ull << 63) % q, r64 = h_mulmod(r63, 2 % q, q), r128 = h_mulmod(r64, r64, q);
        sfold[t].r64 = h_tw(r64, q), sfold[t].r128 = h_tw(r128, q);
        sfold[t].off = q - h_mulmod(r63, r128, q), sfold[t].pad = 0;
    }
    std::vector<uint16_t> pairs;
    for (uint32_t t = 0; t < LK; t++)
        for (uint32_t d = 0; d < tb.beta; d++)
            if (!bx[(size_t)d * LK + t].own) pairs.push_back((uint16_t)(d | (t << 8)));
    tb.pairs = pairs;
    if (tb.d_bx.upload(ctx, bx, "the key switch's extension constants") || tb.d_bxp.upload(ctx, bxp, "the key switch's lift constants") ||
        tb.d_pinv.upload(ctx, pinv, "the key switch's P^-1 table") || tb.d_sfold.upload(ctx, sfold, "the c0 fold's reduction constants"))
        return 1;
    ctx->ext[name] = sp;
    *out = sp.get();
    return 0;
}

int lm_ks_tables_view(lumen_ctx *ctx, lm_ks_view *out) {
    KsTables *tb = nullptr;
    if (int rc = get_tables(ctx, &tb)) return rc;
    out->d_bxp = tb->d_bxp.get();
    out->d_pinv = tb->d_pinv.get();
    out->yscale = &tb->yscale;
    return 0;
}

int lm_launch_pack_v(lumen_ctx *ctx, u64 *y, size_t poly_stride, uint32_t npoly, uint32_t ngroups,
                     uint32_t group_limbs, uint32_t first_mod, uint32_t nlimbs_total) {
    hipLaunchKernelGGL(k_pack_v, dim3(2048), dim3(256), 0, ctx->stream, y, poly_stride, npoly, ngroups, group_limbs,
                       first_mod, nlimbs_total, ctx->logN, ctx->mods);
    LM_HIP(ctx, hipGetLastError());
    return 0;
}

namespace {

static int interleave_work_lists(lumen_ctx *ctx, const std::vector<std::vector<uint32_t>> &lists, size_t expect,
                                 const char *what, std::map<uint32_t, lm_dev<uint32_t>> &cache, uint32_t cache_key,
                                 const uint32_t **out) {
    std::vector<uint32_t> order;
    order.reserve(expect);
    std::vector<size_t> pos(8, 0);
    for (bool any = true; any;) {
        any = false;
        for (uint32_t x = 0; x < 8; x++)
            if (pos[x] < lists[x].size()) {
                order.push_back(lists[x][pos[x]++]);
                any = true;
            }
    }
    LM_CHECK(ctx, order.size() == expect, "%s work list is inconsistent", what);
    lm_dev<uint32_t> d;
    if (int rc = d.upload(ctx, order, "a key-switch work list")) return rc;
    *out = (cache[cache_key] = std::move(d)).get();
    return 0;
}

static int modup_work_list(lumen_ctx *ctx, KsTables *tb, uint32_t B, const uint32_t **out) {
    const uint32_t LM_MODUP_TGROUP = ctx->tune.modup_tgroup;
    LM_SHARED_LOCK(ctx);
    LM_CHECK(ctx, B >= 1 && B <= 65535 && tb->beta <= 255 && tb->nl + ctx->K <= 255,
             "key-switch batch of %u columns (beta %u) does not fit the packed work list", B, tb->beta);
    const uint32_t cache_key = B | (LM_MODUP_TGROUP << 16);
    auto it = tb->d_work.find(cache_key);
    if (it != tb->d_work.end()) {
        *out = it->second.get();
        return 0;
    }
    const uint32_t LK = tb->nl + ctx->K, beta = tb->beta;
    std::vector<std::vector<uint8_t>> need(beta);
    for (uint16_t pr : tb->pairs) need[pr & 0xFF].push_back((uint8_t)(pr >> 8));
    std::vector<std::vector<uint32_t>> lists(8);
    for (uint32_t x = 0; x < 8; x++)
        for (uint32_t t0 = 0; t0 < LK; t0 += LM_MODUP_TGROUP)
            for (uint32_t b = x; b < B; b += 8)
                for (uint32_t d = 0; d < beta; d++)
                    for (uint8_t t : need[d])
                        if (t >= t0 && t < t0 + LM_MODUP_TGROUP) lists[x].push_back(b | (d << 16) | ((uint32_t)t << 24));
    return interleave_work_lists(ctx, lists, (size_t)B * tb->pairs.size(), "extension", tb->d_work, cache_key, out);
}

static int moddown_work_list(lumen_ctx *ctx, KsTables *tb, uint32_t B, const uint32_t **out, bool c1_only = false) {
    const uint32_t LM_MODDOWN_TGROUP = ctx->tune.moddown_tgroup;
    LM_SHARED_LOCK(ctx);
    LM_CHECK(ctx, B >= 1 && 2 * (uint64_t)B <= 65535, "key-switch batch of %u columns does not fit the packed work list", B);
    const uint32_t cache_key = B | (LM_MODDOWN_TGROUP << 17) | (c1_only ? 1u << 31 : 0u);
    auto it = tb->d_work_down.find(cache_key);
    if (it != tb->d_work_down.end()) {
        *out = it->second.get();
        return 0;
    }
    const uint32_t L = tb->nl;
    std::vector<std::vector<uint32_t>> lists(8);
    for (uint32_t x = 0; x < 8; x++)
        for (uint32_t t0 = 0; t0 < L; t0 += LM_MODDOWN_TGROUP)
            for (uint32_t pw = c1_only ? 2 * x + 1 : x; pw < 2 * B; pw += c1_only ? 16 : 8)
                for (uint32_t t = t0; t < std::min<uint32_t>(t0 + LM_MODDOWN_TGROUP, L); t++) lists[x].push_back(pw | (t << 16));
    return interleave_work_lists(ctx, lists, (size_t)(c1_only ? 1 : 2) * B * L, "ModDown", tb->d_work_down, cache_key, out);
}

template <int LOGN>
static uint32_t intt_pack_slots(lumen_ctx *ctx) {
    static const uint32_t v = [&] {
        hipDeviceProp_t prop;
        int per_cu = 0;
        if (hipGetDeviceProperties(&prop, ctx->device) != hipSuccess) return 256u;
        (void)hipFuncSetAttribute(reinterpret_cast<const void *>(&k_intt_pack<LOGN>),
                                  hipFuncAttributeMaxDynamicSharedMemorySize, (int)LM_CU_LDS_BYTES);
        constexpr lm_geom g = lm_geom_lds(LOGN);
        if (hipOccupancyMaxActiveBlocksPerMultiprocessor(&per_cu, k_intt_pack<LOGN>, g.threads, g.lds) != hipSuccess || per_cu < 1) {
            per_cu = (int)std::max<size_t>(1, std::min<size_t>(LM_CU_LDS_BYTES / g.lds, 2048 / g.threads));
        }
        (void)hipGetLastError();
        if (ctx->tune.debug)
            fprintf(stderr, "[lumenos_hip] k_intt_pack<%d>: %d workgroup(s) per CU, %d CUs\n", LOGN, per_cu,
                    prop.multiProcessorCount);
        return (uint32_t)prop.multiProcessorCount * (uint32_t)per_cu;
    }();
    return v;
}
static uint32_t ks_fused_digits(lumen_ctx *ctx, uint32_t B, uint32_t L) {
    if (lm_is_split(ctx->logN)) return 0;
    const long forced = ctx->tune.ks_fused_digits;
    const uint32_t pairs = L / 2;
    if (forced >= 0) return std::min<uint32_t>((uint32_t)forced, pairs);
    uint32_t slots = 0;
    if (lm_for_logn(ctx, ctx->logN, [&](auto n) { return slots = intt_pack_slots<n>(ctx), 0; })) return 0;
    for (uint32_t nf = pairs; nf >= 1; nf--)
        if (((uint64_t)B * nf) % slots == 0) return nf;
    return 0;
}

static int launch_ks_mac(lumen_ctx *ctx, const u64 *ext, const u64 *acc, const u64 *key, u64 *u, uint32_t B, KsTables *tb) {
    const uint32_t L = tb->nl, K = ctx->K, pshift = ctx->L - L, key_beta = (ctx->L + K - 1) / K;
    const dim3 grid(((ctx->N / LM_MAC_VEC + 255) / 256) * (L + K) * ((B + LM_MAC_COLS - 1) / LM_MAC_COLS));
    hipLaunchKernelGGL(k_ks_mac, grid, dim3(256), 0, ctx->stream, ext, acc, key, u, B, L, K, tb->beta, pshift, key_beta, ctx->logN,
                       ctx->mods);
    LM_HIP(ctx, hipGetLastError());
    return 0;
}
static int launch_ks_mac_fold(lumen_ctx *ctx, const u64 *ext, const u64 *acc, const lm_galois_key &gk, u64 *u, u64 *acc_out, uint32_t B,
                              KsTables *tb) {
    const uint32_t L = tb->nl, K = ctx->K, pshift = ctx->L - L, key_beta = (ctx->L + K - 1) / K;
    LM_CHECK(ctx, ctx->N >= 256 && LM_MAC_VEC == 1, "the folded gadget product works on blocks of 256 coefficients");
    const dim3 grid((ctx->N / 256) * (L + K) * ((B + LM_MAC_COLS - 1) / LM_MAC_COLS));
    hipLaunchKernelGGL(k_ks_mac_fold, grid, dim3(256), 0, ctx->stream, ext, acc, gk.d_key.get(), u, B, L, K, tb->beta, pshift, key_beta,
                       ctx->logN, ctx->mods, acc_out, gk.d_index.get(), gk.d_inv_index.get());
    LM_HIP(ctx, hipGetLastError());
    return 0;
}

template <bool ACCUMULATE>
static int launch_moddown(lumen_ctx *ctx, const u64 *in, u64 *out, uint32_t B, const lm_galois_key &gk, KsTables *tb,
                          const KsScratch &s, bool c1_only = false) {
    const uint32_t L = tb->nl, K = ctx->K;
    const uint32_t *work_down = nullptr;
    if (int rc = moddown_work_list(ctx, tb, B, &work_down, c1_only)) return rc;
    const uint32_t items = (c1_only ? 1 : 2) * B * L;
    lm_prof_scope ps(ctx, ACCUMULATE ? "ks_moddown_ntt" : "ks_rotdown_ntt", (uint64_t)items);
    return lm_for_any_logn(ctx, ctx->logN, [&](auto n) {
        constexpr int LN = decltype(n)::value;
        return lm_launch(ctx, ACCUMULATE ? k_moddown_ntt<LN> : k_rotdown_ntt<LN>, lm_geom_fwd(LN), lm_fwd_grid<LN>(items), s.u, in, out, tb->d_bxp.get(), tb->d_pinv.get(),
                         gk.d_index.get(), gk.d_inv_index.get(), work_down, B, L, K, ctx->mods, ctx->sh->tw_fwd.get());
    });
}

}

int rotate_decompose(lumen_ctx *ctx, const u64 *acc, uint32_t B, KsTables *tb, const KsScratch &s) {
    const uint32_t N = ctx->N, L = tb->nl, K = ctx->K, beta = tb->beta;
    const uint32_t pshift = ctx->L - L;
    const uint32_t nf = K == 2 ? ks_fused_digits(ctx, B, L) : 0;
    if (nf) {
        const uint32_t grid = B * nf + B * (L - 2 * nf);
        lm_prof_scope ps(ctx, "ks_intt_c1", (uint64_t)B * L);
        if (int rc = lm_for_logn(ctx, ctx->logN, [&](auto n) {
                return lm_launch(ctx, k_intt_pack<n>, lm_geom_lds(n), grid, acc, s.coef, B, L, nf, ctx->mods, tb->yscale,
                                 ctx->sh->tw_inv.get());
            }))
            return rc;
    } else {
        if (int rc = lm_launch_ntt_strided(ctx, acc + (size_t)L * N, (size_t)2 * L * N, s.coef, (size_t)L * N, B,
                                           lm_map_q(L), true, "ks_intt_c1", &tb->yscale))
            return rc;
    }
    if (K == 2 && nf < beta) {
        lm_prof_scope ps(ctx, "ks_pack_v", (uint64_t)B);
        if (int rc = lm_launch_pack_v(ctx, s.coef + (size_t)2 * nf * N, (size_t)L * N, B, beta - nf, K, 2 * nf, L - 2 * nf)) return rc;
    }
    {
        const uint64_t nb = (uint64_t)B * tb->pairs.size();
        const uint32_t *work = nullptr;
        if (int rc = modup_work_list(ctx, tb, B, &work)) return rc;
        lm_prof_scope ps(ctx, "ks_modup_ntt", nb);
        if (int rc = lm_for_any_logn(ctx, ctx->logN, [&](auto n) {
                return lm_launch(ctx, k_modup_ntt<n>, lm_geom_fwd(n), lm_fwd_grid<n>((uint32_t)nb), s.coef, acc, s.ext, tb->d_bx.get(), B, L, K, beta,
                                 pshift, work, ctx->mods, ctx->sh->tw_fwd.get());
            }))
            return rc;
    }
    return 0;
}

int rotate_product(lumen_ctx *ctx, const u64 *acc, uint32_t B, const lm_galois_key &gk, KsTables *tb, const KsScratch &s) {
    if (int rc = rotate_mac(ctx, acc, B, gk, tb, s)) return rc;
    return rotate_p_to_coef(ctx, s.u, B, tb);
}

int rotate_mac(lumen_ctx *ctx, const u64 *acc, uint32_t B, const lm_galois_key &gk, KsTables *tb, const KsScratch &s) {
    lm_prof_scope ps(ctx, "ks_mac", (uint64_t)B);
    return launch_ks_mac(ctx, s.ext, acc, gk.d_key.get(), s.u, B, tb);
}

int rotate_p_to_coef(lumen_ctx *ctx, u64 *u, uint32_t B, KsTables *tb, bool c1_only) {
    const uint32_t N = ctx->N, L = tb->nl, K = ctx->K;
    u64 *up = u + ks_u_at(c1_only ? 1 : 0, L, B, L, K) * N;
    const size_t pstride = (size_t)(c1_only ? 2 : 1) * K * N;
    const uint32_t npoly = c1_only ? B : B * 2;
    if (int rc = lm_launch_ntt_strided(ctx, up, pstride, up, pstride, npoly, lm_map_p(ctx), true, "ks_intt_p",
                                       &tb->yscale))
        return rc;
    if (K == 2) {
        lm_prof_scope ps(ctx, "ks_pack_v", (uint64_t)B);
        if (int rc = lm_launch_pack_v(ctx, up, pstride, npoly, 1u, K, ctx->L, K)) return rc;
    }
    return 0;
}

int rotate_accumulate(lumen_ctx *ctx, const u64 *acc, u64 *acc_out, uint32_t B, const lm_galois_key &gk,
                      KsTables *tb, const KsScratch &s) {
    if (int rc = rotate_decompose(ctx, acc, B, tb, s)) return rc;
    return rotate_add(ctx, acc, acc_out, B, gk, tb, s);
}

int rotate_add(lumen_ctx *ctx, const u64 *acc, u64 *acc_out, uint32_t B, const lm_galois_key &gk, KsTables *tb, const KsScratch &s) {
    if (int rc = rotate_product(ctx, acc, B, gk, tb, s)) return rc;
    return launch_moddown<true>(ctx, acc, acc_out, B, gk, tb, s);
}

int rotate_store(lumen_ctx *ctx, const u64 *in, u64 *out, uint32_t B, const lm_galois_key &gk, KsTables *tb, const KsScratch &s) {
    return launch_moddown<false>(ctx, in, out, B, gk, tb, s);
}

int rotate_store_c1(lumen_ctx *ctx, const u64 *in, u64 *out, uint32_t B, const lm_galois_key &gk, KsTables *tb, const KsScratch &s) {
    return launch_moddown<false>(ctx, in, out, B, gk, tb, s, true);
}

int rotate_close(lumen_ctx *ctx, const u64 *acc, u64 *coef_out, uint32_t B, const lm_galois_key &gk, uint64_t gal_el,
                 KsTables *tb, const KsScratch &s) {
    if (int rc = rotate_product(ctx, acc, B, gk, tb, s)) return rc;
    const uint32_t *work_down = nullptr;
    if (int rc = moddown_work_list(ctx, tb, B, &work_down)) return rc;
    return ks_close_launch(ctx, acc, coef_out, B, gk, gal_el, tb, s, work_down);
}

#ifndef LM_KS_FOLD_MIN_ROTATIONS
#define LM_KS_FOLD_MIN_ROTATIONS 3
#endif
bool ks_fold_serves(const lumen_ctx *ctx, const KsTables *tb, uint32_t rotations) {
    return ctx->N >= 256 && !lm_is_split(ctx->logN) && ctx->K >= 1 && ctx->K <= 2 && rotations >= LM_KS_FOLD_MIN_ROTATIONS &&
           rotations + tb->lift_bits <= 191;
}

int rotate_add_fold(lumen_ctx *ctx, const u64 *acc, u64 *acc_out, uint32_t B, const lm_galois_key &gk, uint64_t gal_el, KsTables *tb,
                    const KsScratch &s, const u64 *s_in, u64 *s_out) {
    {
        lm_prof_scope ps(ctx, "ks_mac", (uint64_t)B);
        if (int rc = launch_ks_mac_fold(ctx, s.ext, acc, gk, s.u, acc_out, B, tb)) return rc;
    }
    if (int rc = rotate_p_to_coef(ctx, s.u, B, tb)) return rc;
    if (int rc = lift_fold_launch(ctx, s.u, s_in, s_out, B, gal_el, tb)) return rc;
    return launch_moddown<true>(ctx, acc, acc_out, B, gk, tb, s, true);
}

int rotate_close_fold(lumen_ctx *ctx, const u64 *acc, u64 *coef_out, uint32_t B, const lm_galois_key &gk, uint64_t gal_el,
                      KsTables *tb, const KsScratch &s, const u64 *s_in, u64 *s_out) {
    if (int rc = rotate_product(ctx, acc, B, gk, tb, s)) return rc;
    if (int rc = lift_fold_launch(ctx, s.u, s_in, s_out, B, gal_el, tb)) return rc;
    const uint32_t *work_down = nullptr;
    if (int rc = moddown_work_list(ctx, tb, B, &work_down)) return rc;
    return ks_close_launch(ctx, acc, coef_out, B, gk, gal_el, tb, s, work_down, s_out);
}

extern "C" int lumen_ks_mac_probe(lumen_ctx *ctx, uint32_t batch, const void *ext, const void *acc, const void *key,
                                  void *u, uint32_t reps, float *ms_per_launch) {
    LM_CHECK(nullptr, ctx && ms_per_launch, "lumen_ks_mac_probe: NULL argument");
    LM_ENTER(ctx);
    KsTables *tb = nullptr;
    if (int rc = get_tables(ctx, &tb)) return rc;
    const uint32_t N = ctx->N, L = ctx->L, B = batch ? batch : ks_batch(ctx);
    LM_CHECK(ctx, B <= 65535 && reps >= 1 && reps <= 100000, "lumen_ks_mac_probe: batch %u / reps %u out of range", B, reps);
    KsScratch s;
    if (int rc = get_scratch(ctx, B, tb, &s)) return rc;
    if (!acc) acc = lm_scratch(ctx, "ks_acc", (size_t)B * 2 * L * N * 8);
    if (!acc) return 1;
    if (!key) {
        LM_SHARED_LOCK(ctx);
        LM_CHECK(ctx, !ctx->gkeys.empty(), "lumen_ks_mac_probe: no Galois key loaded");
        key = ctx->gkeys.begin()->second.d_key.get();
    }
    const u64 *pe = ext ? (const u64 *)ext : s.ext;
    u64 *pu = u ? (u64 *)u : s.u;
    auto launch = [&] { return launch_ks_mac(ctx, pe, (const u64 *)acc, (const u64 *)key, pu, B, tb); };
    for (int i = 0; i < 3; i++)
        if (int rc = launch()) return rc;
    LM_HIP(ctx, hipEventRecord(ctx->tm0, ctx->stream));
    for (uint32_t i = 0; i < reps; i++)
        if (int rc = launch()) return rc;
    LM_HIP(ctx, hipEventRecord(ctx->tm1, ctx->stream));
    LM_HIP(ctx, hipEventSynchronize(ctx->tm1));
    float ms = 0;
    LM_HIP(ctx, hipEventElapsedTime(&ms, ctx->tm0, ctx->tm1));
    *ms_per_launch = ms / (float)reps;
    return 0;
}
```

### lumenos_amd/csrc/lm_ks_batch.hip

```cpp
#include "lm_ks_host.h"

uint32_t ks_batch(const lumen_ctx *ctx) { return ctx->tune.ks_batch; }

uint32_t ks_lanes(const lumen_ctx *ctx) {
    return ctx->tune.ks_lanes ? ctx->tune.ks_lanes : (ctx->logN <= 13 ? 2 : 1);
}

int check_level_of_chain(lumen_ctx *ctx, const lumen_set *in, const char *what) {
    LM_FULL_WIDTH(ctx, in, what);
    LM_CHECK(ctx, in->nl >= 1 && in->nl <= ctx->L, "%s: set has %u limbs, the chain has %u", what, in->nl, ctx->L);
    return 0;
}

int ks_run_open(lumen_ctx *ctx, uint32_t count, uint32_t nl, uint32_t max_lanes, bool group_acc, KsRun *run) {
    if (int rc = get_tables(ctx, &run->top)) return rc;
    if (int rc = get_tables_at(ctx, nl, &run->tb)) return rc;
    run->Bmax = std::min<uint32_t>(ks_batch(ctx), std::max(count, 1u));
    run->group = group_acc ? std::min<uint32_t>(8 * run->Bmax, std::max(count, 1u)) : std::max(count, 1u);
    run->lanes = std::min(ks_lanes(ctx), max_lanes);
    run->grouped = group_acc;
    run->group_bytes = (size_t)run->group * 2 * ctx->L * ctx->N * 8;
    return 0;
}

int ks_run_scratch(lumen_ctx *ctx, KsRun *run) {
    if (get_scratch(ctx, run->Bmax, run->top, &run->s[0], 0, run->grouped ? &run->acc : nullptr, run->grouped ? run->group_bytes : 0) ||
        (run->lanes > 1 && get_scratch(ctx, run->Bmax, run->top, &run->s[1], 1)))
        return 1;
    return run->grouped && !run->acc ? 1 : 0;
}
```

### lumenos_amd/csrc/lm_ks_host.h

```cpp
#pragma once
#include "lm_ks_dev.h"

struct KsTables {
    lm_dev<bx_t> d_bx;
    lm_dev<bx_t> d_bxp;
    lm_dev<tw_t> d_pinv;
    lm_dev<sfold_t> d_sfold;
    u64 m2_lo = 0, m2_hi = 0;
    uint32_t lift_bits = 0;
    uint32_t nl = 0;
    uint32_t beta = 0;
    lm_ninv_t yscale;
    std::vector<uint16_t> pairs;
    std::map<uint32_t, lm_dev<uint32_t>> d_work;
    std::map<uint32_t, lm_dev<uint32_t>> d_work_down;
};
int get_tables(lumen_ctx *ctx, KsTables **out);
int get_tables_at(lumen_ctx *ctx, uint32_t nl, KsTables **out);

struct KsScratch {
    u64 *coef, *ext, *u, *acc2;
};

int rotate_decompose(lumen_ctx *ctx, const u64 *acc, uint32_t B, KsTables *tb, const KsScratch &s);
int rotate_product(lumen_ctx *ctx, const u64 *acc, uint32_t B, const lm_galois_key &gk, KsTables *tb, const KsScratch &s);
int rotate_mac(lumen_ctx *ctx, const u64 *acc, uint32_t B, const lm_galois_key &gk, KsTables *tb, const KsScratch &s);
int rotate_p_to_coef(lumen_ctx *ctx, u64 *u, uint32_t B, KsTables *tb, bool c1_only = false);
int rotate_add(lumen_ctx *ctx, const u64 *acc, u64 *acc_out, uint32_t B, const lm_galois_key &gk, KsTables *tb, const KsScratch &s);
int rotate_accumulate(lumen_ctx *ctx, const u64 *acc, u64 *acc_out, uint32_t B, const lm_galois_key &gk,
                      KsTables *tb, const KsScratch &s);
int rotate_store(lumen_ctx *ctx, const u64 *in, u64 *out, uint32_t B, const lm_galois_key &gk, KsTables *tb, const KsScratch &s);
int rotate_store_c1(lumen_ctx *ctx, const u64 *in, u64 *out, uint32_t B, const lm_galois_key &gk, KsTables *tb, const KsScratch &s);
int rotate_close(lumen_ctx *ctx, const u64 *acc, u64 *coef_out, uint32_t B, const lm_galois_key &gk, uint64_t gal_el,
                 KsTables *tb, const KsScratch &s);
int ks_close_launch(lumen_ctx *ctx, const u64 *acc, u64 *out, uint32_t B, const lm_galois_key &gk, uint64_t gal_el,
                    KsTables *tb, const KsScratch &s, const uint32_t *work_down, const u64 *fold_s = nullptr);

bool ks_fold_serves(const lumen_ctx *ctx, const KsTables *tb, uint32_t rotations);
inline size_t ks_fold_words(const lumen_ctx *ctx, uint32_t B) { return (size_t)B * 3 * ctx->N; }
int rotate_add_fold(lumen_ctx *ctx, const u64 *acc, u64 *acc_out, uint32_t B, const lm_galois_key &gk, uint64_t gal_el, KsTables *tb,
                    const KsScratch &s, const u64 *s_in, u64 *s_out);
int rotate_close_fold(lumen_ctx *ctx, const u64 *acc, u64 *coef_out, uint32_t B, const lm_galois_key &gk, uint64_t gal_el,
                      KsTables *tb, const KsScratch &s, const u64 *s_in, u64 *s_out);
int lift_fold_launch(lumen_ctx *ctx, const u64 *u, const u64 *s_in, u64 *s_out, uint32_t B, uint64_t gal_el, KsTables *tb);
int get_scratch(lumen_ctx *ctx, uint32_t B, KsTables *tb, KsScratch *s, int lane = 0, u64 **group_acc = nullptr,
                size_t group_acc_bytes = 0);

int upload_ptT(lumen_ctx *ctx, const uint64_t *pt, uint32_t nl, u64 **out);
int launch_pt_prepare(lumen_ctx *ctx, const u64 *raw, u64 *ptM, uint32_t nl, uint32_t np);
int launch_mul_plain(lumen_ctx *ctx, const u64 *ct, u64 *out, const u64 *ptT, size_t words, uint32_t nl,
                     uint32_t ncts);

struct KsRun;
int lazy_blocks(lumen_ctx *ctx, const KsRun &run, u64 **lazy);
int identity_tables(lumen_ctx *ctx, std::shared_ptr<lm_galois_key> *out);
int lazy_close(lumen_ctx *ctx, const u64 *cur, u64 *out, u64 *lazy, uint32_t B, KsTables *tb, const KsScratch &s);

std::shared_ptr<lm_galois_key> lm_relin_key(lumen_ctx *ctx);
int ks_find_key(lumen_ctx *ctx, uint64_t gal_el, const lm_galois_key **gk);
int check_level_of_chain(lumen_ctx *ctx, const lumen_set *in, const char *what);
uint32_t ks_batch(const lumen_ctx *ctx);
uint32_t ks_lanes(const lumen_ctx *ctx);
struct LaneGuard {
    lumen_ctx *ctx;
    hipStream_t saved;
    LaneGuard(lumen_ctx *c, int lane) : ctx(c), saved(c->stream) {
        if (lane) ctx->stream = ctx->stream2;
    }
    ~LaneGuard() { ctx->stream = saved; }
};

struct KsRun {
    KsTables *top = nullptr, *tb = nullptr;
    uint32_t Bmax = 0, group = 0, lanes = 1;
    bool grouped = false;
    size_t group_bytes = 0;
    KsScratch s[2] = {};
    u64 *acc = nullptr;
};
int ks_run_open(lumen_ctx *ctx, uint32_t count, uint32_t nl, uint32_t max_lanes, bool group_acc, KsRun *run);
int ks_run_scratch(lumen_ctx *ctx, KsRun *run);
template <class Batch, class Group>
int ks_run(lumen_ctx *ctx, const KsRun &run, uint32_t count, size_t ctw, Batch &&batch, Group &&end_of_group) {
    for (uint32_t g0 = 0; g0 < count; g0 += run.group) {
        const uint32_t gn = std::min(run.group, count - g0);
        if (run.lanes > 1) {
            LM_HIP(ctx, hipEventRecord(ctx->ev_fork, ctx->stream));
            LM_HIP(ctx, hipStreamWaitEvent(ctx->stream2, ctx->ev_fork, 0));
        }
        uint32_t lane = 0;
        for (uint32_t first = 0; first < gn; first += run.Bmax, lane = (lane + 1) % run.lanes) {
            const uint32_t B = std::min(run.Bmax, gn - first);
            LaneGuard guard(ctx, (int)lane);
            if (int rc = batch(g0, first, B, run.s[lane], run.acc ? run.acc + (size_t)first * ctw : nullptr)) return rc;
        }
        if (run.lanes > 1) {
            LM_HIP(ctx, hipEventRecord(ctx->ev_join, ctx->stream2));
            LM_HIP(ctx, hipStreamWaitEvent(ctx->stream, ctx->ev_join, 0));
        }
        if (int rc = end_of_group(g0, gn)) return rc;
    }
    return 0;
}
template <class Batch>
int ks_run(lumen_ctx *ctx, const KsRun &run, uint32_t count, size_t ctw, Batch &&batch) {
    return ks_run(ctx, run, count, ctw, batch, [](uint32_t, uint32_t) { return 0; });
}
```

### lumenos_amd/csrc/lm_ks_mac_kernel.h

```cpp
#if LM_KS_MAC_FOLD
__global__ __launch_bounds__(256) void k_ks_mac_fold(const u64 *__restrict__ ext, const u64 *__restrict__ acc,
                                                     const u64 *__restrict__ key, u64 *__restrict__ u, uint32_t B,
                                                     uint32_t L, uint32_t K, uint32_t beta, uint32_t pshift,
                                                     uint32_t key_beta, uint32_t logN, lm_mods mods,
                                                     u64 *__restrict__ acc_out, const uint32_t *__restrict__ index,
                                                     const uint32_t *__restrict__ inv_index) {
#else
__global__ __launch_bounds__(256) void k_ks_mac(const u64 *__restrict__ ext, const u64 *__restrict__ acc,
                                                const u64 *__restrict__ key, u64 *__restrict__ u, uint32_t B,
                                                uint32_t L, uint32_t K, uint32_t beta, uint32_t pshift,
                                                uint32_t key_beta, uint32_t logN, lm_mods mods) {
#endif
    typedef mac_vec<LM_MAC_VEC> vec;
    const uint32_t N = 1u << logN, LK = L + K;
    const uint32_t G = (B + LM_MAC_COLS - 1) / LM_MAC_COLS, per_limb = N / (256 * LM_MAC_VEC) ? N / (256 * LM_MAC_VEC) : 1;
    const uint32_t slices = per_limb * LK;
    uint32_t slice, z;
    if (slices % 8 == 0) {
        const uint32_t xcd = blockIdx.x & 7, j = blockIdx.x >> 3;
        z = j % G;
        slice = (j / G) * 8 + xcd;
    } else {
        z = blockIdx.x % G;
        slice = blockIdx.x / G;
    }
    const uint32_t i = ((slice % per_limb) * 256 + threadIdx.x) * LM_MAC_VEC;
    const uint32_t t = LK - 1 - slice / per_limb;
    const uint32_t mt = ks_mod_at(t, L, pshift);
    const uint32_t b0 = z * LM_MAC_COLS;
    if (i >= N) return;
    const mod_t md = mods.m[mt];
    const uint32_t own = t < L ? t / K : 0xFFFFFFFFu;
    mac_acc a0[LM_MAC_COLS][LM_MAC_VEC], a1[LM_MAC_COLS][LM_MAC_VEC];
#pragma unroll
    for (int c = 0; c < LM_MAC_COLS; c++)
#pragma unroll
        for (int e = 0; e < LM_MAC_VEC; e++) a0[c][e].clear(), a1[c][e].clear();
    struct digit_t {
        vec k0, k1, x[LM_MAC_COLS];
    };
    auto fetch = [&](uint32_t d) {
        digit_t g;
        g.k0 = vec::load(key + ks_key_at(d, 0, mt, key_beta) * N + i);
        g.k1 = vec::load(key + ks_key_at(d, 1, mt, key_beta) * N + i);
#pragma unroll
        for (int c = 0; c < LM_MAC_COLS; c++) {
            const uint32_t bc = b0 + c < B ? b0 + c : B - 1;
            g.x[c] = d == own ? vec::load(acc + ((size_t)(bc * 2 + 1) * L + t) * N + i)
                              : vec::load_once(ext + ks_ext_at(bc, d, t, B, beta) * N + i);
        }
        return g;
    };
    constexpr int PF = LM_MAC_PREFETCH;
    digit_t q[PF + 1];
#pragma unroll
    for (int j = 0; j < PF; j++)
        if ((uint32_t)j < beta) q[j] = fetch(j);
    for (uint32_t d0 = 0; d0 < beta; d0 += PF + 1) {
#pragma unroll
        for (int j = 0; j <= PF; j++) {
            const uint32_t d = d0 + j;
            if (d < beta) {
                if (d + PF < beta) q[(j + PF) % (PF + 1)] = fetch(d + PF);
#pragma unroll
                for (int c = 0; c < LM_MAC_COLS; c++)
#pragma unroll
                    for (int e = 0; e < LM_MAC_VEC; e++) mac2(a0[c][e], a1[c][e], q[j].x[c].v[e], q[j].k0.v[e], q[j].k1.v[e]);
            }
        }
    }
#if LM_KS_MAC_FOLD
    u64 u0[LM_MAC_COLS];
#endif
#pragma unroll
    for (int c = 0; c < LM_MAC_COLS; c++) {
        if (b0 + c < B) {
            u64 *o = u + ks_u_at((b0 + c) * 2, t, B, L, K) * N + i, *o1 = u + ks_u_at((b0 + c) * 2 + 1, t, B, L, K) * N + i;
            vec r0, r1;
#pragma unroll
            for (int e = 0; e < LM_MAC_VEC; e++) {
                u64 lo, hi;
                a0[c][e].value(lo, hi);
                r0.v[e] = lm_mont_reduce_wide(lo, hi, md.q, md.qneg, md.qinv64, beta);
                a1[c][e].value(lo, hi);
                r1.v[e] = lm_mont_reduce_wide(lo, hi, md.q, md.qneg, md.qinv64, beta);
            }
#if LM_KS_MAC_FOLD
            if (t >= L) r0.store(o);
            u0[c] = r0.v[0];
#else
            r0.store(o);
#endif
            r1.store(o1);
        }
    }
#if LM_KS_MAC_FOLD
    {
        static_assert(LM_MAC_VEC == 1, "the fold parks one coefficient per thread");
        __shared__ u64 park[LM_MAC_COLS][256];
        if (t < L) {
            const uint32_t i0 = i - threadIdx.x;
            const uint32_t j = (inv_index[i0] & ~255u) + threadIdx.x;
            const uint32_t src = index[j] & 255u;
            u64 aj[LM_MAC_COLS];
#pragma unroll
            for (int c = 0; c < LM_MAC_COLS; c++)
                if (b0 + c < B) {
                    const u64 *a = acc + ((size_t)(b0 + c) * 2 * L + t) * N;
                    park[c][threadIdx.x] = a[i] + u0[c];
                    aj[c] = a[j];
                }
            __syncthreads();
#pragma unroll
            for (int c = 0; c < LM_MAC_COLS; c++)
                if (b0 + c < B)
                    acc_out[((size_t)(b0 + c) * 2 * L + t) * N + j] = lm_csub(lm_csub(aj[c] + park[c][src], 4 * md.q), 2 * md.q);
        }
    }
#endif
}
```

### lumenos_amd/csrc/lm_ks_scratch.hip

```cpp
#include "lm_ks_host.h"
#include "lm_placement.h"

namespace {

struct ProfOff {
    lumen_ctx *ctx;
    bool saved;
    explicit ProfOff(lumen_ctx *c) : ctx(c), saved(c->prof) { ctx->prof = false; }
    ~ProfOff() { ctx->prof = saved; }
};
struct EventPair {
    lumen_ctx *ctx;
    hipEvent_t e0, e1;
    explicit EventPair(lumen_ctx *c) : ctx(c), e0(lm_ev_get(c)), e1(lm_ev_get(c)) {}
    ~EventPair() { ctx->ev_pool.push_back(e0), ctx->ev_pool.push_back(e1); }
};

}

int get_scratch(lumen_ctx *ctx, uint32_t B, KsTables *tb, KsScratch *s, int lane, u64 **group_acc, size_t group_acc_bytes) {
    const size_t N = ctx->N, L = ctx->L, LK = ctx->L + ctx->K, beta = tb->beta;
    const char *names[2][5] = {{"ks_coef", "ks_ext", "ks_u", "ks_acc2", "ks_acc"}, {"ks_coef_b", "ks_ext_b", "ks_u_b", "ks_acc2_b", "ks_acc"}};
    const int NB = group_acc ? 5 : 4;
    const size_t bytes[5] = {(size_t)B * L * N * 8, (size_t)B * beta * LK * N * 8, (size_t)B * 2 * LK * N * 8, (size_t)B * 2 * L * N * 8,
                             std::max(group_acc_bytes, (size_t)B * 2 * L * N * 8)};
    u64 *dummy = nullptr;
    u64 **slot[5] = {&s->coef, &s->ext, &s->u, &s->acc2, group_acc ? group_acc : &dummy};
    const uint32_t Kc = ctx->tune.ks_placement;
    std::vector<lm_place_buf> bufs;
    bool have = true;
    for (int c = 0; c < NB; c++) {
        auto it = ctx->scratch.find(names[lane][c]);
        const bool there = it != ctx->scratch.end() && it->second && it->second.count() >= bytes[c];
        bufs.push_back({bytes[c], there ? it->second.get() : nullptr, c == 4 ? 4u : Kc});
        have = have && there;
    }
    const lm_galois_key *gk = nullptr;
    {
        LM_SHARED_LOCK(ctx);
        if (!ctx->gkeys.empty()) gk = &ctx->gkeys.begin()->second;
    }
    const std::shared_ptr<lm_galois_key> rlk = gk ? nullptr : lm_relin_key(ctx);
    if (!gk) gk = rlk.get();
    auto plain = [&]() -> int {
        bool ok = true;
        for (int c = 0; c < NB; c++) ok = (*slot[c] = (u64 *)lm_scratch(ctx, names[lane][c], bytes[c])) != nullptr && ok;
        return ok ? 0 : 1;
    };
    if (have || Kc < 2 || bytes[1] < ((size_t)64 << 20) || !gk || !gk->d_key) return plain();
    {
        size_t free_b = 0, total_b = 0;
        (void)hipMemGetInfo(&free_b, &total_b);
        lm_dev<u64> probe_acc;
        if (!group_acc) (void)probe_acc.alloc(ctx, bytes[3] / 8, "the placement's probe accumulator");
        lm_placement place(bufs, [](void *p) { hipFree(p); });
        const bool drew = place.draw(Kc, free_b, [&](size_t c) {
            void *p = nullptr;
            return hipMalloc(&p, bytes[c]) == hipSuccess ? p : nullptr;
        });
        (void)hipGetLastError();
        if (drew && (group_acc || probe_acc)) {
            int rc;
            {
                ProfOff quiet(ctx);
                EventPair ev(ctx);
                auto eval = [&](const size_t *pick, float *ms) -> int {
                    KsScratch t;
                    t.coef = (u64 *)place.block(0, pick[0]), t.ext = (u64 *)place.block(1, pick[1]), t.u = (u64 *)place.block(2, pick[2]),
                    t.acc2 = (u64 *)place.block(3, pick[3]);
                    u64 *a0 = group_acc ? (u64 *)place.block(4, pick[4]) : probe_acc.get();
                    u64 *a1 = group_acc ? a0 + (bytes[4] - bytes[3]) / 8 : a0;
                    for (int r = 0; r < 3; r++) {
                        if (r == 1) LM_HIP(ctx, hipEventRecord(ev.e0, ctx->stream));
                        u64 *a = r == 2 ? a1 : a0;
                        if (int e = rotate_accumulate(ctx, a, t.acc2, B, *gk, tb, t)) return e;
                        if (int e = rotate_accumulate(ctx, t.acc2, a, B, *gk, tb, t)) return e;
                    }
                    LM_HIP(ctx, hipEventRecord(ev.e1, ctx->stream));
                    LM_HIP(ctx, hipEventSynchronize(ev.e1));
                    LM_HIP(ctx, hipEventElapsedTime(ms, ev.e0, ev.e1));
                    return 0;
                };
                rc = place.descend(group_acc ? std::vector<int>{2, 1, 4, 3, 0} : std::vector<int>{2, 1, 3, 0}, eval);
            }
            if (rc) {
                lm_sync_all(ctx);
                return rc;
            }
            if (ctx->tune.debug)
                fprintf(stderr, "[lumenos_hip] key-switch scratch placement (lane %d, %u columns): %zu / %zu / %zu candidates for u / ext / the group "
                                "accumulator, 4 rotations of the first draw %.3f ms, of the chosen blocks %.3f ms\n", lane, B, place.count(2),
                        place.count(1), NB == 5 ? place.count(4) : (size_t)0, place.first, place.best_all);
            LM_HIP(ctx, hipStreamSynchronize(ctx->stream));
            for (int c = 0; c < NB; c++) {
                void *chosen = place.take(c);
                if (!bufs[c].fixed) lm_scratch_adopt(ctx, names[lane][c], chosen, bytes[c]);
                *slot[c] = (u64 *)chosen;
            }
            return 0;
        }
    }
    return plain();
}
```

Baseline: 1.657 s.

## Pair key-switch batches into double-width launches with split ext buffers at LogN 14

Adds a pair mode, on by default at logN 14 with a single lane, where the key-switch loop takes two batches of columns at a time. Coef, u and accumulator scratch are sized for twice the batch width, and the extended-basis buffer is split into two half-size allocations. The modup NTT runs as two launches, one per half, while the MAC kernels pick the right ext half per column and run once over the doubled batch. The aim is fewer launches and more work per launch to fill the GPU, at the cost of more scratch memory and extra indexing in the MAC kernel.

```diff
diff --git a/lumenos_amd/csrc/lm_common.h b/lumenos_amd/csrc/lm_common.h
--- a/lumenos_amd/csrc/lm_common.h
+++ b/lumenos_amd/csrc/lm_common.h
@@ -64,6 +64,7 @@
 struct lm_tuning {
     uint32_t ks_batch = 64;
     uint32_t ks_lanes = 0;
+    int32_t ks_pair = -1;
     int32_t ks_fused_digits = -1;
     uint32_t ks_close_fused = 1;
     uint32_t ks_c0_fold = 1;
diff --git a/lumenos_amd/csrc/lm_ctx.hip b/lumenos_amd/csrc/lm_ctx.hip
--- a/lumenos_amd/csrc/lm_ctx.hip
+++ b/lumenos_amd/csrc/lm_ctx.hip
@@ -174,6 +174,9 @@
     } else if (n == "LUMEN_KS_LANES") {
         if (!in(0, 2)) return 2;
         t.ks_lanes = (uint32_t)v;
+    } else if (n == "LUMEN_KS_PAIR") {
+        if (v > 2) return 2;
+        t.ks_pair = v >= 0 ? (int32_t)v : -1;
     } else if (n == "LUMEN_KS_FUSED_DIGITS") {
         if (v > LM_MAX_LIMBS) return 2;
         t.ks_fused_digits = v >= 0 ? (int32_t)v : -1;
@@ -209,7 +212,7 @@
     return 0;
 }
 static void tuning_from_env(lm_tuning &t) {
-    for (const char *n : {"LUMEN_KS_BATCH", "LUMEN_KS_LANES", "LUMEN_KS_FUSED_DIGITS", "LUMEN_KS_CLOSE_FUSED", "LUMEN_KS_C0_FOLD", "LUMEN_DEBUG",
+    for (const char *n : {"LUMEN_KS_BATCH", "LUMEN_KS_LANES", "LUMEN_KS_PAIR", "LUMEN_KS_FUSED_DIGITS", "LUMEN_KS_CLOSE_FUSED", "LUMEN_KS_C0_FOLD", "LUMEN_DEBUG",
                           "LUMEN_MODUP_TGROUP", "LUMEN_MODDOWN_TGROUP", "LUMEN_KS_PLACEMENT", "LUMEN_BATCH_CHUNKS", "LUMEN_DOT_PAIRS", "LUMEN_DOT_PARTS"}) {
         const char *e = getenv(n);
         if (e && *e && tuning_set(t, n, atol(e)))
diff --git a/lumenos_amd/csrc/lm_innersum.hip b/lumenos_amd/csrc/lm_innersum.hip
--- a/lumenos_amd/csrc/lm_innersum.hip
+++ b/lumenos_amd/csrc/lm_innersum.hip
@@ -105,7 +105,7 @@
 
 
 int lazy_blocks(lumen_ctx *ctx, const KsRun &run, u64 **lazy) {
-    const size_t bytes = (size_t)run.Bmax * 2 * (ctx->L + ctx->K) * ctx->N * 8;
+    const size_t bytes = (size_t)run.Bcap() * 2 * (ctx->L + ctx->K) * ctx->N * 8;
     lazy[0] = (u64 *)lm_scratch(ctx, "ks_lazy", bytes);
     lazy[1] = run.lanes > 1 ? (u64 *)lm_scratch(ctx, "ks_lazy_b", bytes) : lazy[0];
     return lazy[0] && lazy[1] ? 0 : 1;
@@ -198,7 +198,7 @@
         LM_CHECK(ctx, is_plain(ctx, batch, n), "InnerSum length %u is not a power of two <= N", n);
     }
     KsRun run;
-    if (int rc = ks_run_open(ctx, in->count, in->nl, is_plain(ctx, batch, n) ? 1 : 2, false, &run)) return rc;
+    if (int rc = ks_run_open(ctx, in->count, in->nl, is_plain(ctx, batch, n) ? 1 : 2, false, &run, true)) return rc;
     SumPlan plan;
     if (in->count)
         if (int rc = sum_plan(ctx, batch, n, &plan)) return rc;
@@ -230,7 +230,7 @@
         LM_CHECK(ctx, is_plain(ctx, 1, rows), "rows=%u is not a power of two <= N", rows);
     }
     KsRun run;
-    if (int rc = ks_run_open(ctx, matrix->count, matrix->nl, 2, true, &run)) return rc;
+    if (int rc = ks_run_open(ctx, matrix->count, matrix->nl, 2, true, &run, true)) return rc;
     SumPlan plan;
     if (matrix->count)
         if (int rc = sum_plan(ctx, 1, rows, &plan)) return rc;
@@ -256,7 +256,7 @@
     }
     u64 *fold_s[2] = {nullptr, nullptr};
     if (close && ctx->tune.ks_c0_fold && ks_fold_serves(ctx, run.tb, plan.cnt)) {
-        const size_t bytes = 2 * ks_fold_words(ctx, run.Bmax) * 8;
+        const size_t bytes = 2 * ks_fold_words(ctx, run.Bcap()) * 8;
         fold_s[0] = (u64 *)lm_scratch(ctx, "ks_fold_s", bytes);
         fold_s[1] = run.lanes > 1 ? (u64 *)lm_scratch(ctx, "ks_fold_s_b", bytes) : fold_s[0];
         if (!fold_s[0] || !fold_s[1]) return 1;
diff --git a/lumenos_amd/csrc/lm_keyswitch.hip b/lumenos_amd/csrc/lm_keyswitch.hip
--- a/lumenos_amd/csrc/lm_keyswitch.hip
+++ b/lumenos_amd/csrc/lm_keyswitch.hip
@@ -603,21 +603,24 @@
     return 0;
 }
 
-static int launch_ks_mac(lumen_ctx *ctx, const u64 *ext, const u64 *acc, const u64 *key, u64 *u, uint32_t B, KsTables *tb) {
+static int launch_ks_mac(lumen_ctx *ctx, const u64 *ext, const u64 *ext1, uint32_t Bh, const u64 *acc, const u64 *key, u64 *u, uint32_t B,
+                         KsTables *tb) {
     const uint32_t L = tb->nl, K = ctx->K, pshift = ctx->L - L, key_beta = (ctx->L + K - 1) / K;
+    LM_CHECK(ctx, Bh >= 1 && Bh <= B && (Bh == B || (ext1 && B <= 2 * Bh)), "gadget product: %u columns do not fit blocks of %u", B, Bh);
     const dim3 grid(((ctx->N / LM_MAC_VEC + 255) / 256) * (L + K) * ((B + LM_MAC_COLS - 1) / LM_MAC_COLS));
-    hipLaunchKernelGGL(k_ks_mac, grid, dim3(256), 0, ctx->stream, ext, acc, key, u, B, L, K, tb->beta, pshift, key_beta, ctx->logN,
-                       ctx->mods);
+    hipLaunchKernelGGL(k_ks_mac, grid, dim3(256), 0, ctx->stream, ext, ext1 ? ext1 : ext, Bh, acc, key, u, B, L, K, tb->beta, pshift, key_beta,
+                       ctx->logN, ctx->mods);
     LM_HIP(ctx, hipGetLastError());
     return 0;
 }
-static int launch_ks_mac_fold(lumen_ctx *ctx, const u64 *ext, const u64 *acc, const lm_galois_key &gk, u64 *u, u64 *acc_out, uint32_t B,
-                              KsTables *tb) {
+static int launch_ks_mac_fold(lumen_ctx *ctx, const u64 *ext, const u64 *ext1, uint32_t Bh, const u64 *acc, const lm_galois_key &gk, u64 *u,
+                              u64 *acc_out, uint32_t B, KsTables *tb) {
     const uint32_t L = tb->nl, K = ctx->K, pshift = ctx->L - L, key_beta = (ctx->L + K - 1) / K;
     LM_CHECK(ctx, ctx->N >= 256 && LM_MAC_VEC == 1, "the folded gadget product works on blocks of 256 coefficients");
+    LM_CHECK(ctx, Bh >= 1 && Bh <= B && (Bh == B || (ext1 && B <= 2 * Bh)), "gadget product: %u columns do not fit blocks of %u", B, Bh);
     const dim3 grid((ctx->N / 256) * (L + K) * ((B + LM_MAC_COLS - 1) / LM_MAC_COLS));
-    hipLaunchKernelGGL(k_ks_mac_fold, grid, dim3(256), 0, ctx->stream, ext, acc, gk.d_key.get(), u, B, L, K, tb->beta, pshift, key_beta,
-                       ctx->logN, ctx->mods, acc_out, gk.d_index.get(), gk.d_inv_index.get());
+    hipLaunchKernelGGL(k_ks_mac_fold, grid, dim3(256), 0, ctx->stream, ext, ext1 ? ext1 : ext, Bh, acc, gk.d_key.get(), u, B, L, K, tb->beta, pshift,
+                       key_beta, ctx->logN, ctx->mods, acc_out, gk.d_index.get(), gk.d_inv_index.get());
     LM_HIP(ctx, hipGetLastError());
     return 0;
 }
@@ -661,15 +664,21 @@
         if (int rc = lm_launch_pack_v(ctx, s.coef + (size_t)2 * nf * N, (size_t)L * N, B, beta - nf, K, 2 * nf, L - 2 * nf)) return rc;
     }
     {
-        const uint64_t nb = (uint64_t)B * tb->pairs.size();
-        const uint32_t *work = nullptr;
-        if (int rc = modup_work_list(ctx, tb, B, &work)) return rc;
-        lm_prof_scope ps(ctx, "ks_modup_ntt", nb);
-        if (int rc = lm_for_any_logn(ctx, ctx->logN, [&](auto n) {
-                return lm_launch(ctx, k_modup_ntt<n>, lm_geom_fwd(n), lm_fwd_grid<n>((uint32_t)nb), s.coef, acc, s.ext, tb->d_bx.get(), B, L, K, beta,
-                                 pshift, work, ctx->mods, ctx->sh->tw_fwd.get());
-            }))
-            return rc;
+        const lm_ks_ext_plan plan = lm_ks_ext_launches(B, s.half, s.second_first);
+        for (uint32_t k = 0; k < plan.n; k++) {
+            const lm_ks_ext_launch &h = plan.at[k];
+            const uint64_t nb = (uint64_t)h.count * tb->pairs.size();
+            const uint32_t *work = nullptr;
+            if (int rc = modup_work_list(ctx, tb, h.count, &work)) return rc;
+            const u64 *coef_h = s.coef + (size_t)h.first * L * N, *acc_h = acc + (size_t)h.first * 2 * L * N;
+            u64 *ext_h = h.block ? s.ext1 : s.ext;
+            lm_prof_scope ps(ctx, "ks_modup_ntt", nb);
+            if (int rc = lm_for_any_logn(ctx, ctx->logN, [&](auto n) {
+                    return lm_launch(ctx, k_modup_ntt<n>, lm_geom_fwd(n), lm_fwd_grid<n>((uint32_t)nb), coef_h, acc_h, ext_h, tb->d_bx.get(), plan.layout, L, K,
+                                     beta, pshift, work, ctx->mods, ctx->sh->tw_fwd.get());
+                }))
+                return rc;
+        }
     }
     return 0;
 }
@@ -681,7 +690,7 @@
 
 int rotate_mac(lumen_ctx *ctx, const u64 *acc, uint32_t B, const lm_galois_key &gk, KsTables *tb, const KsScratch &s) {
     lm_prof_scope ps(ctx, "ks_mac", (uint64_t)B);
-    return launch_ks_mac(ctx, s.ext, acc, gk.d_key.get(), s.u, B, tb);
+    return launch_ks_mac(ctx, s.ext, s.ext1, lm_ks_ext_launches(B, s.half).layout, acc, gk.d_key.get(), s.u, B, tb);
 }
 
 int rotate_p_to_coef(lumen_ctx *ctx, u64 *u, uint32_t B, KsTables *tb, bool c1_only) {
@@ -738,7 +747,7 @@
                     const KsScratch &s, const u64 *s_in, u64 *s_out) {
     {
         lm_prof_scope ps(ctx, "ks_mac", (uint64_t)B);
-        if (int rc = launch_ks_mac_fold(ctx, s.ext, acc, gk, s.u, acc_out, B, tb)) return rc;
+        if (int rc = launch_ks_mac_fold(ctx, s.ext, s.ext1, lm_ks_ext_launches(B, s.half).layout, acc, gk, s.u, acc_out, B, tb)) return rc;
     }
     if (int rc = rotate_p_to_coef(ctx, s.u, B, tb)) return rc;
     if (int rc = lift_fold_launch(ctx, s.u, s_in, s_out, B, gal_el, tb)) return rc;
@@ -773,7 +782,7 @@
     }
     const u64 *pe = ext ? (const u64 *)ext : s.ext;
     u64 *pu = u ? (u64 *)u : s.u;
-    auto launch = [&] { return launch_ks_mac(ctx, pe, (const u64 *)acc, (const u64 *)key, pu, B, tb); };
+    auto launch = [&] { return launch_ks_mac(ctx, pe, nullptr, B, (const u64 *)acc, (const u64 *)key, pu, B, tb); };
     for (int i = 0; i < 3; i++)
         if (int rc = launch()) return rc;
     LM_HIP(ctx, hipEventRecord(ctx->tm0, ctx->stream));
diff --git a/lumenos_amd/csrc/lm_ks_batch.hip b/lumenos_amd/csrc/lm_ks_batch.hip
--- a/lumenos_amd/csrc/lm_ks_batch.hip
+++ b/lumenos_amd/csrc/lm_ks_batch.hip
@@ -6,26 +6,33 @@
     return ctx->tune.ks_lanes ? ctx->tune.ks_lanes : (ctx->logN <= 13 ? 2 : 1);
 }
 
+uint32_t ks_pair(const lumen_ctx *ctx) {
+    return ctx->tune.ks_pair >= 0 ? (uint32_t)ctx->tune.ks_pair : (ctx->logN == 14 ? 1 : 0);
+}
+
 int check_level_of_chain(lumen_ctx *ctx, const lumen_set *in, const char *what) {
     LM_FULL_WIDTH(ctx, in, what);
     LM_CHECK(ctx, in->nl >= 1 && in->nl <= ctx->L, "%s: set has %u limbs, the chain has %u", what, in->nl, ctx->L);
     return 0;
 }
 
-int ks_run_open(lumen_ctx *ctx, uint32_t count, uint32_t nl, uint32_t max_lanes, bool group_acc, KsRun *run) {
+int ks_run_open(lumen_ctx *ctx, uint32_t count, uint32_t nl, uint32_t max_lanes, bool group_acc, KsRun *run, bool may_pair) {
     if (int rc = get_tables(ctx, &run->top)) return rc;
     if (int rc = get_tables_at(ctx, nl, &run->tb)) return rc;
     run->Bmax = std::min<uint32_t>(ks_batch(ctx), std::max(count, 1u));
     run->group = group_acc ? std::min<uint32_t>(8 * run->Bmax, std::max(count, 1u)) : std::max(count, 1u);
     run->lanes = std::min(ks_lanes(ctx), max_lanes);
+    run->pair = may_pair && ks_pair(ctx) && run->lanes == 1 && count > run->Bmax;
     run->grouped = group_acc;
     run->group_bytes = (size_t)run->group * 2 * ctx->L * ctx->N * 8;
     return 0;
 }
 
 int ks_run_scratch(lumen_ctx *ctx, KsRun *run) {
-    if (get_scratch(ctx, run->Bmax, run->top, &run->s[0], 0, run->grouped ? &run->acc : nullptr, run->grouped ? run->group_bytes : 0) ||
+    if (get_scratch(ctx, run->Bmax, run->top, &run->s[0], 0, run->grouped ? &run->acc : nullptr, run->grouped ? run->group_bytes : 0,
+                    run->pair) ||
         (run->lanes > 1 && get_scratch(ctx, run->Bmax, run->top, &run->s[1], 1)))
         return 1;
+    run->s[0].second_first = run->pair && ks_pair(ctx) == 2;
     return run->grouped && !run->acc ? 1 : 0;
 }
diff --git a/lumenos_amd/csrc/lm_ks_host.h b/lumenos_amd/csrc/lm_ks_host.h
--- a/lumenos_amd/csrc/lm_ks_host.h
+++ b/lumenos_amd/csrc/lm_ks_host.h
@@ -1,5 +1,6 @@
 #pragma once
 #include "lm_ks_dev.h"
+#include "lm_ks_pair.h"
 
 struct KsTables {
     lm_dev<bx_t> d_bx;
@@ -20,6 +21,9 @@
 
 struct KsScratch {
     u64 *coef, *ext, *u, *acc2;
+    u64 *ext1 = nullptr;
+    uint32_t half = 0;
+    bool second_first = false;
 };
 
 int rotate_decompose(lumen_ctx *ctx, const u64 *acc, uint32_t B, KsTables *tb, const KsScratch &s);
@@ -44,7 +48,7 @@
                       KsTables *tb, const KsScratch &s, const u64 *s_in, u64 *s_out);
 int lift_fold_launch(lumen_ctx *ctx, const u64 *u, const u64 *s_in, u64 *s_out, uint32_t B, uint64_t gal_el, KsTables *tb);
 int get_scratch(lumen_ctx *ctx, uint32_t B, KsTables *tb, KsScratch *s, int lane = 0, u64 **group_acc = nullptr,
-                size_t group_acc_bytes = 0);
+                size_t group_acc_bytes = 0, bool pair = false);
 
 int upload_ptT(lumen_ctx *ctx, const uint64_t *pt, uint32_t nl, u64 **out);
 int launch_pt_prepare(lumen_ctx *ctx, const u64 *raw, u64 *ptM, uint32_t nl, uint32_t np);
@@ -61,6 +65,7 @@
 int check_level_of_chain(lumen_ctx *ctx, const lumen_set *in, const char *what);
 uint32_t ks_batch(const lumen_ctx *ctx);
 uint32_t ks_lanes(const lumen_ctx *ctx);
+uint32_t ks_pair(const lumen_ctx *ctx);
 struct LaneGuard {
     lumen_ctx *ctx;
     hipStream_t saved;
@@ -73,12 +78,13 @@
 struct KsRun {
     KsTables *top = nullptr, *tb = nullptr;
     uint32_t Bmax = 0, group = 0, lanes = 1;
-    bool grouped = false;
+    bool grouped = false, pair = false;
+    uint32_t Bcap() const { return pair ? 2 * Bmax : Bmax; }
     size_t group_bytes = 0;
     KsScratch s[2] = {};
     u64 *acc = nullptr;
 };
-int ks_run_open(lumen_ctx *ctx, uint32_t count, uint32_t nl, uint32_t max_lanes, bool group_acc, KsRun *run);
+int ks_run_open(lumen_ctx *ctx, uint32_t count, uint32_t nl, uint32_t max_lanes, bool group_acc, KsRun *run, bool may_pair = false);
 int ks_run_scratch(lumen_ctx *ctx, KsRun *run);
 template <class Batch, class Group>
 int ks_run(lumen_ctx *ctx, const KsRun &run, uint32_t count, size_t ctw, Batch &&batch, Group &&end_of_group) {
@@ -89,8 +95,8 @@
             LM_HIP(ctx, hipStreamWaitEvent(ctx->stream2, ctx->ev_fork, 0));
         }
         uint32_t lane = 0;
-        for (uint32_t first = 0; first < gn; first += run.Bmax, lane = (lane + 1) % run.lanes) {
-            const uint32_t B = std::min(run.Bmax, gn - first);
+        for (uint32_t first = 0, B = 0; first < gn; first += B, lane = (lane + 1) % run.lanes) {
+            B = lm_ks_take(run.Bmax, run.pair, gn - first);
             LaneGuard guard(ctx, (int)lane);
             if (int rc = batch(g0, first, B, run.s[lane], run.acc ? run.acc + (size_t)first * ctw : nullptr)) return rc;
         }
diff --git a/lumenos_amd/csrc/lm_ks_mac_kernel.h b/lumenos_amd/csrc/lm_ks_mac_kernel.h
--- a/lumenos_amd/csrc/lm_ks_mac_kernel.h
+++ b/lumenos_amd/csrc/lm_ks_mac_kernel.h
@@ -1,12 +1,14 @@
 #if LM_KS_MAC_FOLD
-__global__ __launch_bounds__(256) void k_ks_mac_fold(const u64 *__restrict__ ext, const u64 *__restrict__ acc,
+__global__ __launch_bounds__(256) void k_ks_mac_fold(const u64 *__restrict__ ext, const u64 *__restrict__ ext1, uint32_t Bh,
+                                                     const u64 *__restrict__ acc,
                                                      const u64 *__restrict__ key, u64 *__restrict__ u, uint32_t B,
                                                      uint32_t L, uint32_t K, uint32_t beta, uint32_t pshift,
                                                      uint32_t key_beta, uint32_t logN, lm_mods mods,
                                                      u64 *__restrict__ acc_out, const uint32_t *__restrict__ index,
                                                      const uint32_t *__restrict__ inv_index) {
 #else
-__global__ __launch_bounds__(256) void k_ks_mac(const u64 *__restrict__ ext, const u64 *__restrict__ acc,
+__global__ __launch_bounds__(256) void k_ks_mac(const u64 *__restrict__ ext, const u64 *__restrict__ ext1, uint32_t Bh,
+                                                const u64 *__restrict__ acc,
                                                 const u64 *__restrict__ key, u64 *__restrict__ u, uint32_t B,
                                                 uint32_t L, uint32_t K, uint32_t beta, uint32_t pshift,
                                                 uint32_t key_beta, uint32_t logN, lm_mods mods) {
@@ -46,8 +48,9 @@
 #pragma unroll
         for (int c = 0; c < LM_MAC_COLS; c++) {
             const uint32_t bc = b0 + c < B ? b0 + c : B - 1;
+            const u64 *xb = bc < Bh ? ext : ext1;
             g.x[c] = d == own ? vec::load(acc + ((size_t)(bc * 2 + 1) * L + t) * N + i)
-                              : vec::load_once(ext + ks_ext_at(bc, d, t, B, beta) * N + i);
+                              : vec::load_once(xb + ks_ext_at(bc < Bh ? bc : bc - Bh, d, t, Bh, beta) * N + i);
         }
         return g;
     };
diff --git a/lumenos_amd/csrc/lm_ks_pair.h b/lumenos_amd/csrc/lm_ks_pair.h
--- /dev/null
+++ b/lumenos_amd/csrc/lm_ks_pair.h
@@ -0,0 +1,30 @@
+#pragma once
+#include <algorithm>
+#include <cstdint>
+
+inline uint32_t lm_ks_take(uint32_t Bmax, bool pair, uint32_t left) {
+    return pair && left > Bmax ? std::min(2 * Bmax, left) : std::min(Bmax, left);
+}
+
+struct lm_ks_ext_launch {
+    uint32_t first, count, block;
+};
+struct lm_ks_ext_plan {
+    uint32_t layout = 0;
+    uint32_t n = 0;
+    lm_ks_ext_launch at[2];
+};
+inline lm_ks_ext_plan lm_ks_ext_launches(uint32_t B, uint32_t half, bool second_first = false) {
+    lm_ks_ext_plan p;
+    if (!half || B <= half) {
+        p.layout = B, p.n = 1;
+        p.at[0] = {0, B, 0};
+        return p;
+    }
+    p.layout = half, p.n = 2;
+    p.at[second_first ? 1 : 0] = {0, half, 0};
+    p.at[second_first ? 0 : 1] = {half, B - half, 1};
+    return p;
+}
+inline uint32_t lm_ks_ext_block(uint32_t b, uint32_t layout) { return b < layout ? 0 : 1; }
+inline uint32_t lm_ks_ext_local(uint32_t b, uint32_t layout) { return b < layout ? b : b - layout; }
diff --git a/lumenos_amd/csrc/lm_ks_scratch.hip b/lumenos_amd/csrc/lm_ks_scratch.hip
--- a/lumenos_amd/csrc/lm_ks_scratch.hip
+++ b/lumenos_amd/csrc/lm_ks_scratch.hip
@@ -18,21 +18,29 @@
 
 }
 
-int get_scratch(lumen_ctx *ctx, uint32_t B, KsTables *tb, KsScratch *s, int lane, u64 **group_acc, size_t group_acc_bytes) {
+int get_scratch(lumen_ctx *ctx, uint32_t B, KsTables *tb, KsScratch *s, int lane, u64 **group_acc, size_t group_acc_bytes, bool pair) {
     const size_t N = ctx->N, L = ctx->L, LK = ctx->L + ctx->K, beta = tb->beta;
-    const char *names[2][5] = {{"ks_coef", "ks_ext", "ks_u", "ks_acc2", "ks_acc"}, {"ks_coef_b", "ks_ext_b", "ks_u_b", "ks_acc2_b", "ks_acc"}};
-    const int NB = group_acc ? 5 : 4;
-    const size_t bytes[5] = {(size_t)B * L * N * 8, (size_t)B * beta * LK * N * 8, (size_t)B * 2 * LK * N * 8, (size_t)B * 2 * L * N * 8,
-                             std::max(group_acc_bytes, (size_t)B * 2 * L * N * 8)};
+    LM_CHECK(ctx, !pair || lane == 0, "a pair of key-switch batches runs on the first lane");
+    enum { COEF, EXT, U, ACC2, ACC, EXT1, NBUF };
+    const char *names[2][NBUF] = {{"ks_coef", "ks_ext", "ks_u", "ks_acc2", "ks_acc", "ks_ext_b"}, {"ks_coef_b", "ks_ext_b", "ks_u_b", "ks_acc2_b", "ks_acc", ""}};
+    const uint32_t Bt = pair ? 2 * B : B;
+    const size_t bytes[NBUF] = {(size_t)Bt * L * N * 8, (size_t)B * beta * LK * N * 8, (size_t)Bt * 2 * LK * N * 8, (size_t)Bt * 2 * L * N * 8,
+                                std::max(group_acc_bytes, (size_t)Bt * 2 * L * N * 8), (size_t)B * beta * LK * N * 8};
     u64 *dummy = nullptr;
-    u64 **slot[5] = {&s->coef, &s->ext, &s->u, &s->acc2, group_acc ? group_acc : &dummy};
+    u64 **slot[NBUF] = {&s->coef, &s->ext, &s->u, &s->acc2, group_acc ? group_acc : &dummy, &s->ext1};
+    std::vector<int> ids = {COEF, EXT, U, ACC2};
+    if (group_acc) ids.push_back(ACC);
+    if (pair) ids.push_back(EXT1);
+    int at[NBUF] = {-1, -1, -1, -1, -1, -1};
+    for (size_t k = 0; k < ids.size(); k++) at[ids[k]] = (int)k;
+    s->ext1 = nullptr, s->half = pair ? B : 0, s->second_first = false;
     const uint32_t Kc = ctx->tune.ks_placement;
     std::vector<lm_place_buf> bufs;
     bool have = true;
-    for (int c = 0; c < NB; c++) {
+    for (int c : ids) {
         auto it = ctx->scratch.find(names[lane][c]);
         const bool there = it != ctx->scratch.end() && it->second && it->second.count() >= bytes[c];
-        bufs.push_back({bytes[c], there ? it->second.get() : nullptr, c == 4 ? 4u : Kc});
+        bufs.push_back({bytes[c], there ? it->second.get() : nullptr, c == ACC ? 4u : Kc});
         have = have && there;
     }
     const lm_galois_key *gk = nullptr;
@@ -44,19 +52,19 @@
     if (!gk) gk = rlk.get();
     auto plain = [&]() -> int {
         bool ok = true;
-        for (int c = 0; c < NB; c++) ok = (*slot[c] = (u64 *)lm_scratch(ctx, names[lane][c], bytes[c])) != nullptr && ok;
+        for (int c : ids) ok = (*slot[c] = (u64 *)lm_scratch(ctx, names[lane][c], bytes[c])) != nullptr && ok;
         return ok ? 0 : 1;
     };
-    if (have || Kc < 2 || bytes[1] < ((size_t)64 << 20) || !gk || !gk->d_key) return plain();
+    if (have || Kc < 2 || bytes[EXT] < ((size_t)64 << 20) || !gk || !gk->d_key) return plain();
     {
         size_t free_b = 0, total_b = 0;
         (void)hipMemGetInfo(&free_b, &total_b);
         lm_dev<u64> probe_acc;
-        if (!group_acc) (void)probe_acc.alloc(ctx, bytes[3] / 8, "the placement's probe accumulator");
+        if (!group_acc) (void)probe_acc.alloc(ctx, bytes[ACC2] / 8, "the placement's probe accumulator");
         lm_placement place(bufs, [](void *p) { hipFree(p); });
-        const bool drew = place.draw(Kc, free_b, [&](size_t c) {
+        const bool drew = place.draw(Kc, free_b, [&](size_t k) {
             void *p = nullptr;
-            return hipMalloc(&p, bytes[c]) == hipSuccess ? p : nullptr;
+            return hipMalloc(&p, bytes[ids[k]]) == hipSuccess ? p : nullptr;
         });
         (void)hipGetLastError();
         if (drew && (group_acc || probe_acc)) {
@@ -65,36 +73,41 @@
                 ProfOff quiet(ctx);
                 EventPair ev(ctx);
                 auto eval = [&](const size_t *pick, float *ms) -> int {
+                    auto blk = [&](int c) { return (u64 *)place.block((size_t)at[c], pick[at[c]]); };
                     KsScratch t;
-                    t.coef = (u64 *)place.block(0, pick[0]), t.ext = (u64 *)place.block(1, pick[1]), t.u = (u64 *)place.block(2, pick[2]),
-                    t.acc2 = (u64 *)place.block(3, pick[3]);
-                    u64 *a0 = group_acc ? (u64 *)place.block(4, pick[4]) : probe_acc.get();
-                    u64 *a1 = group_acc ? a0 + (bytes[4] - bytes[3]) / 8 : a0;
+                    t.coef = blk(COEF), t.ext = blk(EXT), t.u = blk(U), t.acc2 = blk(ACC2);
+                    if (pair) t.ext1 = blk(EXT1), t.half = B;
+                    u64 *a0 = group_acc ? blk(ACC) : probe_acc.get();
+                    u64 *a1 = group_acc ? a0 + (bytes[ACC] - bytes[ACC2]) / 8 : a0;
                     for (int r = 0; r < 3; r++) {
                         if (r == 1) LM_HIP(ctx, hipEventRecord(ev.e0, ctx->stream));
                         u64 *a = r == 2 ? a1 : a0;
-                        if (int e = rotate_accumulate(ctx, a, t.acc2, B, *gk, tb, t)) return e;
-                        if (int e = rotate_accumulate(ctx, t.acc2, a, B, *gk, tb, t)) return e;
+                        if (int e = rotate_accumulate(ctx, a, t.acc2, Bt, *gk, tb, t)) return e;
+                        if (int e = rotate_accumulate(ctx, t.acc2, a, Bt, *gk, tb, t)) return e;
                     }
                     LM_HIP(ctx, hipEventRecord(ev.e1, ctx->stream));
                     LM_HIP(ctx, hipEventSynchronize(ev.e1));
                     LM_HIP(ctx, hipEventElapsedTime(ms, ev.e0, ev.e1));
                     return 0;
                 };
-                rc = place.descend(group_acc ? std::vector<int>{2, 1, 4, 3, 0} : std::vector<int>{2, 1, 3, 0}, eval);
+                std::vector<int> order;
+                for (int c : {U, EXT, EXT1, ACC, ACC2, COEF})
+                    if (at[c] >= 0) order.push_back(at[c]);
+                rc = place.descend(order, eval);
             }
             if (rc) {
                 lm_sync_all(ctx);
                 return rc;
             }
             if (ctx->tune.debug)
-                fprintf(stderr, "[lumenos_hip] key-switch scratch placement (lane %d, %u columns): %zu / %zu / %zu candidates for u / ext / the group "
-                                "accumulator, 4 rotations of the first draw %.3f ms, of the chosen blocks %.3f ms\n", lane, B, place.count(2),
-                        place.count(1), NB == 5 ? place.count(4) : (size_t)0, place.first, place.best_all);
+                fprintf(stderr, "[lumenos_hip] key-switch scratch placement (lane %d, %u columns%s): %zu / %zu / %zu candidates for u / ext / the group "
+                                "accumulator, 4 rotations of the first draw %.3f ms, of the chosen blocks %.3f ms\n", lane, Bt, pair ? ", a pair" : "",
+                        place.count((size_t)at[U]), place.count((size_t)at[EXT]), group_acc ? place.count((size_t)at[ACC]) : (size_t)0, place.first,
+                        place.best_all);
             LM_HIP(ctx, hipStreamSynchronize(ctx->stream));
-            for (int c = 0; c < NB; c++) {
-                void *chosen = place.take(c);
-                if (!bufs[c].fixed) lm_scratch_adopt(ctx, names[lane][c], chosen, bytes[c]);
+            for (int c : ids) {
+                void *chosen = place.take((size_t)at[c]);
+                if (!bufs[(size_t)at[c]].fixed) lm_scratch_adopt(ctx, names[lane][c], chosen, bytes[c]);
                 *slot[c] = (u64 *)chosen;
             }
             return 0;
```

New measurement: 1.634 s (median of 6 runs). 1.4% less time.
